# Stanford-ILIAD/PantheonRL

Hardware: AMD Instinct MI355X
Metric: env-steps/sec (all agents) Overcooked-simple PPO self-play (higher is better)
Workload: dtype f32; 1 GPU; OvercookedMultiEnv-v0 layout=simple, PPO self-play (two independent PPO learners per GPU), synthetic (n_envs, n_steps, obs_dim) rollouts; n_envs=1024, n_steps=128, obs_dim=62, features=62, n_logits=6, batch_size=32768, n_epochs=10, agents_per_gpu=2, parallelism=2 agent(s) per gpu x1 gpu(s) = 2 learners (single process), launch_mode=graph, gemm_mode=2, action_masks=none, rollout=scripted, rollout_requested=scripted

## Files before the change

### include/pantheon_hip.h

```cpp
#ifndef PANTHEON_HIP_H
#define PANTHEON_HIP_H

#ifdef __cplusplus
extern "C" {
#endif

#define PH_ABI_VERSION 7
#define PH_HIDDEN 64
#define PH_MAX_COMP 256
#define PH_MAX_LOGITS 64
#define PH_MAX_BOX_ACT 16
#define PH_NSTAT 8
#define PH_MOD_MAX 8
#define PH_MAX_RANKS 16

#define PH_SPACE_BOX 0
#define PH_SPACE_DISCRETE 1

typedef struct ph_ctx ph_ctx;

typedef struct ph_space {
  int kind;
  int n;
  int nvec[PH_MAX_COMP];
// ... 50 lines not shown
int ph_ctx_create(int device, ph_ctx **out );
int ph_ctx_destroy(ph_ctx *ctx);
int ph_ctx_set_stream(ph_ctx *ctx, void *hip_stream );
int ph_ctx_sync(ph_ctx *ctx);
int ph_graph_begin(ph_ctx *ctx);
int ph_graph_end(ph_ctx *ctx, int *graph_id_out );
int ph_graph_launch(ph_ctx *ctx, int graph_id);
int ph_graph_nodes(ph_ctx *ctx, int graph_id, int *nodes_out );
int ph_ctx_set_rng_epoch(ph_ctx *ctx, unsigned long long *epoch_dev );
int ph_rng_epoch_advance(ph_ctx *ctx);
int ph_debug_set_profile_buffer(ph_ctx *ctx, long long *stamps_dev);
int ph_debug_weight_image_mismatches(ph_ctx *ctx, const ph_spec *spec, const float *params, int *mismatches);
int ph_set_exclusive_device(ph_ctx *ctx, int exclusive);
int ph_ctx_step_errors(ph_ctx *ctx, unsigned int *count_out );
int ph_timer_start(ph_ctx *ctx);
int ph_timer_stop(ph_ctx *ctx, float *ms_out );

int ph_layout_of(const ph_spec *spec , ph_layout *out );
int ph_debug_split_tables(const ph_spec *spec, int *slab_map, int *image_map, int *eligible);
int ph_debug_split_oh_tables(const ph_spec *spec, int *slab_map, int *image_map, int *slab_len_out, int *image_elems_out,
                             int *eligible);

int ph_buffer_add(ph_ctx *ctx, const ph_spec *spec, const ph_rollout *rb, int pos, const float *obs ,
                  const float *actions , const float *episode_start ,
                  const float *values , const float *log_probs );
int ph_buffer_add_reward(ph_ctx *ctx, const ph_rollout *rb, int pos, const float *reward ,
                         const unsigned char *env_mask );
int ph_buffer_add_reward_const(ph_ctx *ctx, const ph_rollout *rb, int pos, float reward);
#define PH_JOINT_MATCH_BONUS 0
#define PH_JOINT_RPS 1
int ph_ctx_set_joint_reward_rule(ph_ctx *ctx, int rule);

int ph_buffer_add_reward_joint(ph_ctx *ctx, const ph_rollout *rb, int pos, const float *base_reward ,
                               const int *joint_actions, int n_seats, int seat, const int *partner_seat ,
                               float bonus);
int ph_roundrobin_env_step(ph_ctx *ctx, const int *joint_actions, int *partnerid, const float *base_reward,
                           const float *done, float *reward_out, int *alt_action_out, float *next_block, int block_ld,
                           int n_partners, float bonus, int n);
typedef struct ph_rr_link {
  int n_partners, rank;
  int n, block_ld;
  void *area[PH_MAX_RANKS];
  unsigned long long *error;
  unsigned long long timeout_cycles;
} ph_rr_link;
typedef struct ph_rr_ego {
  const ph_spec *spec;
  const float *params;
  const float *obs_seq;
  const float *base_reward_seq;
  const float *done_seq;
  float *blocks;
  int *partnerid;
  float *rewards;
  int *alt_actions;
  int *partner_trace;
  const float *episode_start0;
  unsigned long long seed, counter0;
  float *values, *log_probs;
  const ph_rollout *rb;
  float bonus;
} ph_rr_ego;
typedef struct ph_rr_partner {
  const ph_spec *spec;
  const float *params;
  float *obs_scratch;
  float *es_scratch;
  unsigned char *can_scratch;
  int *pos;
  unsigned char *boundary, *term, *open, *prev_mask;
  unsigned long long seed, counter0;
  int *actions;
  float *values, *log_probs;
  const ph_rollout *rb;
} ph_rr_partner;
int ph_rr_area_bytes(int n_partners, int n, int block_ld, size_t *bytes_out );
int ph_roundrobin_ego_iteration(ph_ctx *ctx, const ph_rr_link *link, const ph_rr_ego *ego, int T, unsigned long long iteration);
int ph_roundrobin_partner_iteration(ph_ctx *ctx, const ph_rr_link *link, const ph_rr_partner *partner, int T,
                                    unsigned long long iteration);
int ph_buffer_reset(ph_ctx *ctx, const ph_spec *spec, const ph_rollout *rb);

int ph_gae(ph_ctx *ctx, const ph_rollout *rb, const float *last_values , const float *dones ,
           double gamma, double gae_lambda, int mode);

int ph_policy_forward(ph_ctx *ctx, const ph_spec *spec, const float *params, const float *obs, int n,
                      const unsigned char *action_mask, const float *uniforms, const float *given_actions,
                      unsigned long long seed, unsigned long long counter, int deterministic, int *actions_i32,
                      float *actions_f32, float *values, float *log_probs, float *entropy, float *logits,
                      const ph_rollout *rb, int pos, const float *episode_start_in, const float *pending_reward,
                      int gemm_mode);

int ph_policy_act_host(ph_ctx *ctx, const ph_spec *spec, const float *params, const float *obs_host, int n,
                       const float *episode_start_host, unsigned long long seed, unsigned long long counter,
                       int deterministic, int *actions_host, float *values_host, float *log_probs_host,
                       const ph_rollout *rb, int pos, int gemm_mode);

typedef struct ph_step_call {
  const ph_spec *spec;
  const float *params;
  const float *obs;
  int n;
  const unsigned char *action_mask;
  unsigned long long seed, counter;
  int deterministic;
  int *actions_i32;
  float *values;
  float *log_probs;
  const ph_rollout *rb;
  int pos;
  const float *episode_start_in;
  const float *pending_reward;
  const int *joint_actions;
  int n_seats, seat;
  const int *partner_seat;
  float bonus;
} ph_step_call;
#define PH_STEP_FIX_ILLEGAL 2
#define PH_STEP_MASK_ENV_ONLY 4
int ph_policy_step_multi(ph_ctx *ctx, int n_calls, const ph_step_call *calls );

#define PH_COMM_ID_BYTES 128
int ph_comm_unique_id(unsigned char *id_out );
int ph_comm_init(ph_ctx *ctx, const unsigned char *id , int world, int rank);
int ph_comm_destroy(ph_ctx *ctx);
int ph_all_gather_i32(ph_ctx *ctx, const int *local , int *joint , int count);
int ph_selfplay_rollout(ph_ctx *ctx, int n_calls, const ph_step_call *calls , int T,
                        const int *local, int *joint, int count);

#define PH_IPC_HANDLE_BYTES 64
typedef struct ph_p2p {
  int world, rank, count, T;
  int *joint[2][PH_MAX_RANKS];
  unsigned long long *flags[PH_MAX_RANKS];
  unsigned long long *ll[PH_MAX_RANKS];
  int ll_slots;
  const unsigned long long *epoch;
  unsigned long long *error;
  unsigned long long timeout_cycles;
} ph_p2p;
int ph_p2p_alloc(ph_ctx *ctx, size_t bytes, void **ptr_out, unsigned char *handle_out );
int ph_p2p_open(ph_ctx *ctx, const unsigned char *handle , void **ptr_out);
int ph_p2p_close(ph_ctx *ctx, void *ptr);
int ph_p2p_free(ph_ctx *ctx, void *ptr);
int ph_p2p_push(ph_ctx *ctx, const ph_p2p *x, const int *local, int t);
int ph_p2p_wait(ph_ctx *ctx, const ph_p2p *x, int t);
int ph_p2p_ll_push(ph_ctx *ctx, const ph_p2p *x, const int *local, int t);
int ph_p2p_ll_unpack(ph_ctx *ctx, const ph_p2p *x, int t);
int ph_selfplay_rollout_p2p(ph_ctx *ctx, int n_calls, const ph_step_call *calls , int T,
                            const int *local, const ph_p2p *x);

typedef struct ph_rollout_call {
  const ph_spec *spec;
  const float *params;
  const float *obs_seq;
  const float *rew_seq;
  const float *done_seq;
  const unsigned char *mask_seq;
  int n;
  const float *episode_start0;
  unsigned long long seed, counter0;
  int mask_mode;
  int *actions_i32;
  float *values;
  float *log_probs;
  const ph_rollout *rb;
  int n_seats, seat;
// ... 460 lines not shown
```

### pantheonrl_amd/_native.py

```python
from __future__ import annotations

import ctypes as C
import os
from typing import Optional, Sequence

PH_HIDDEN = 64
PH_MAX_COMP = 256
PH_MAX_LOGITS = 64
PH_MAX_BOX_ACT = 16
PH_NSTAT = 8
PH_SPACE_BOX = 0
PH_SPACE_DISCRETE = 1
STAT_NAMES = ("policy_loss", "value_loss", "entropy_loss", "clip_fraction", "approx_kl", "loss", "grad_norm", "applied")

_HERE = os.path.dirname(os.path.abspath(__file__))
LIB_PATH = os.environ.get("PANTHEON_HIP_LIB") or os.path.join(_HERE, "csrc", "libpantheon_hip.so")


class NativeError(RuntimeError):
    """Raised for any non-zero status from the C ABI (message from ph_last_error)."""


class PhSpace(C.Structure):
    _fields_ = [("kind", C.c_int), ("n", C.c_int), ("nvec", C.c_int * PH_MAX_COMP)]
# ... 191 lines not shown
                ("log_probs", C.c_void_p), ("seed", C.c_ulonglong)]


class PhLiarPool(C.Structure):
    _fields_ = [("n", C.c_int), ("spec", C.POINTER(PhSpec)),
                ("hands", C.c_void_p), ("history", C.c_void_p), ("nmoves", C.c_void_p), ("ego_first", C.c_void_p),
                ("dice_seed", C.c_ulonglong), ("probegostart", C.c_float),
                ("ego_params", C.c_void_p), ("ego_rb", C.POINTER(PhRollout)), ("ego_actions", C.c_void_p),
                ("ego_values", C.c_void_p), ("ego_log_probs", C.c_void_p), ("ego_episode_start", C.c_void_p),
                ("ego_seed", C.c_ulonglong),
                ("members", C.POINTER(PhPoolMember)), ("n_members", C.c_int), ("partnerid", C.c_void_p),
                ("resample", C.c_int), ("pool_seed", C.c_ulonglong),
                ("alt_actions", C.c_void_p), ("alt_acted", C.c_void_p),
                ("obs_ego", C.c_void_p), ("obs_alt", C.c_void_p), ("episodes", C.c_void_p),
                ("obs_next", C.c_void_p), ("rew1", C.c_void_p), ("rew2", C.c_void_p), ("es_alt", C.c_void_p),
                ("done1", C.c_void_p), ("done2", C.c_void_p), ("running", C.c_void_p), ("can", C.c_void_p),
                ("alt_opens", C.c_void_p), ("ego_opens", C.c_void_p), ("done", C.c_void_p)]


XPLAY_NSTAT = 4


class PhLiarXplay(C.Structure):
    _fields_ = [("n", C.c_int), ("spec", C.POINTER(PhSpec)),
                ("hands", C.c_void_p), ("history", C.c_void_p), ("nmoves", C.c_void_p), ("ego_first", C.c_void_p),
                ("dice_seed", C.c_ulonglong), ("probegostart", C.c_float),
                ("members", C.POINTER(PhPoolMember)), ("n_members", C.c_int),
                ("pairs", C.POINTER(C.c_int)), ("n_pairs", C.c_int), ("episodes_per_table", C.c_int),
                ("ego_id", C.c_void_p), ("alt_id", C.c_void_p),
                ("ego_actions", C.c_void_p), ("alt_actions", C.c_void_p),
                ("obs_ego", C.c_void_p), ("obs_alt", C.c_void_p),
                ("games", C.c_void_p), ("playing", C.c_void_p), ("tables_left", C.c_void_p),
                ("ep_return", C.c_void_p), ("ep_length", C.c_void_p), ("returns", C.c_void_p), ("lengths", C.c_void_p),
                ("obs_next", C.c_void_p), ("rew1", C.c_void_p), ("rew2", C.c_void_p),
                ("done1", C.c_void_p), ("done2", C.c_void_p), ("running", C.c_void_p),
                ("alt_opens", C.c_void_p), ("ego_opens", C.c_void_p), ("done", C.c_void_p)]


class PhLiarRecord(C.Structure):
    _fields_ = [("n", C.c_int), ("cap", C.c_int), ("rows", C.c_void_p), ("member", C.c_void_p),
                ("count", C.c_void_p), ("count_alt", C.c_void_p), ("dropped", C.c_void_p), ("pending", C.c_void_p)]


RECORD_ROW = 33

EPISODE_NSTAT = 4


class PhEpisodeScan(C.Structure):
    _fields_ = [("rb", C.POINTER(PhRollout)), ("T", C.c_int), ("last_dones", C.c_void_p), ("carry_return", C.c_void_p),
                ("carry_length", C.c_void_p), ("carry_valid", C.c_void_p), ("n_members", C.c_int), ("member", C.c_void_p),
                ("resample", C.c_int), ("pool_seed", C.c_ulonglong), ("counter0", C.c_ulonglong), ("stats", C.c_void_p)]


SIGNATURES = {
    "ph_abi_version": [],
    "ph_roundrobin_env_step": [_vp, _vp, _vp, _vp, _vp, _vp, _vp, _vp, _i, _i, C.c_float, _i],
    "ph_last_error": [],
    "ph_device_count": [C.POINTER(_i)],
    "ph_ctx_create": [_i, C.POINTER(_vp)],
    "ph_ctx_destroy": [_vp],
    "ph_ctx_set_stream": [_vp, _vp],
    "ph_ctx_sync": [_vp],
    "ph_graph_begin": [_vp],
    "ph_graph_end": [_vp, C.POINTER(_i)],
    "ph_graph_launch": [_vp, _i],
    "ph_graph_nodes": [_vp, _i, C.POINTER(C.c_int)],
    "ph_ctx_set_rng_epoch": [_vp, _vp],
    "ph_rng_epoch_advance": [_vp],
    "ph_debug_set_profile_buffer": [_vp, _vp],
    "ph_set_exclusive_device": [_vp, _i],
    "ph_ctx_step_errors": [_vp, C.POINTER(C.c_uint)],
    "ph_debug_weight_image_mismatches": [_vp, C.POINTER(PhSpec), _vp, C.POINTER(C.c_int)],
    "ph_timer_start": [_vp],
    "ph_timer_stop": [_vp, C.POINTER(C.c_float)],
    "ph_layout_of": [C.POINTER(PhSpec), C.POINTER(PhLayout)],
    "ph_debug_split_tables": [C.POINTER(PhSpec), C.POINTER(C.c_int), C.POINTER(C.c_int), C.POINTER(C.c_int)],
    "ph_debug_split_oh_tables": [C.POINTER(PhSpec), _vp, _vp, C.POINTER(_i), C.POINTER(_i), C.POINTER(_i)],
    "ph_buffer_add": [_vp, C.POINTER(PhSpec), C.POINTER(PhRollout), _i, _vp, _vp, _vp, _vp, _vp],
    "ph_buffer_add_reward": [_vp, C.POINTER(PhRollout), _i, _vp, _vp],
    "ph_buffer_add_reward_joint": [_vp, C.POINTER(PhRollout), _i, _vp, _vp, _i, _i, _vp, C.c_float],
    "ph_buffer_reset": [_vp, C.POINTER(PhSpec), C.POINTER(PhRollout)],
    "ph_gae": [_vp, C.POINTER(PhRollout), _vp, _vp, _d, _d, _i],
    "ph_policy_forward": [_vp, C.POINTER(PhSpec), _vp, _vp, _i, _vp, _vp, _vp, _ull, _ull, _i, _vp, _vp, _vp, _vp, _vp,
                          _vp, C.POINTER(PhRollout), _i, _vp, _vp, _i],
    "ph_ctx_set_joint_reward_rule": [_vp, _i],
    "ph_adapmult_layout_of": [C.POINTER(PhSpec), _i, _vp],
    "ph_adapmult_forward": [_vp, C.POINTER(PhSpec), _i, _vp, _vp, _i, _vp, _vp, _vp, _ull, _ull, _i, _vp, _vp, _vp, _vp, _vp,
                            _vp, C.POINTER(PhRollout), _i, _vp],
    "ph_adapmult_minibatch_grad": [_vp, C.POINTER(PhSpec), _i, _vp, C.POINTER(PhRollout), C.POINTER(PhPpoHyper), _vp, _i, _vp, _vp,
                                   _vp],
    "ph_adapmult_train": [_vp, C.POINTER(PhSpec), _i, C.POINTER(PhOptState), C.POINTER(PhRollout), C.POINTER(PhPpoHyper), _i, _i,
                          _vp, _ull, _vp, _vp],
    "ph_policy_act_host": [_vp, C.POINTER(PhSpec), _vp, _vp, _i, _vp, _ull, _ull, _i, _vp, _vp, _vp, C.POINTER(PhRollout), _i, _i],
    "ph_buffer_add_reward_const": [_vp, C.POINTER(PhRollout), _i, C.c_float],
    "ph_policy_step_multi": [_vp, _i, C.POINTER(PhStepCall)],
    "ph_policy_forward_ragged": [_vp, C.POINTER(PhSpec), _vp, _vp, _vp, _ull, _ull, _i, _vp, _vp, _vp, C.POINTER(PhRollout),
                                 _vp, _vp, _vp],
    "ph_buffer_add_reward_ragged": [_vp, C.POINTER(PhRollout), _vp, _vp, _vp],
    "ph_ragged_advance": [_vp, C.POINTER(PhRollout), _vp, _vp],
    "ph_buffer_compact_columns": [_vp, C.POINTER(PhSpec), C.POINTER(PhRollout), C.POINTER(PhRollout), _vp, _i],
    "ph_fix_illegal_actions": [_vp, _vp, _vp, _i, _i],
    "ph_rps_step": [_vp, _vp, _vp, _vp, _vp, _i],
    "ph_liar_step": [_vp, _vp, _vp, _vp, _vp, _vp, _vp, _vp, _vp, _vp, _i],
    "ph_liar_reset": [_vp, _vp, _vp, _vp, _vp, _vp, _ull, _ull, C.c_float, _i],
    "ph_liar_obs": [_vp, _vp, _vp, _vp, _vp, _vp, _vp, _i],
    "ph_liar_selfplay_step": [_vp, C.POINTER(PhLiarSelfPlay), _i, _ull, _i],
    "ph_liar_selfplay_rollout": [_vp, C.POINTER(PhLiarSelfPlay), _i, _i, _ull],
    "ph_pool_forward": [_vp, C.POINTER(PhSpec), C.POINTER(PhPoolMember), _i, _vp, _vp, _vp, _ull, _vp, _vp, _i],
    "ph_liar_default_actions": [_vp, _vp, _vp, _vp, _i],
    "ph_liar_pool_step": [_vp, C.POINTER(PhLiarPool), _i, _ull, _i],
    "ph_liar_xplay_step": [_vp, C.POINTER(PhLiarXplay), _ull, _i],
    "ph_xplay_stats": [_vp, _vp, _vp, _vp, _i, _i, _i, _vp],
    "ph_episode_stats": [_vp, C.POINTER(PhEpisodeScan)],
    "ph_liar_record_attach": [_vp, C.POINTER(PhLiarRecord)],
    "ph_liar_record_export": [_vp, C.POINTER(PhLiarRecord), _i, _vp, _vp, _vp, C.c_longlong],
    "ph_block_reset": [_vp, _i, _vp, _vp, _ull, _ull, _i],
    "ph_block_step": [_vp, _i, _vp, _vp, _i, _vp, _vp, _vp, _vp, _i],
    "ph_block_obs": [_vp, _i, _vp, _i, _vp, _vp, _i],
    "ph_block_selfplay_step": [_vp, C.POINTER(PhBlockSelfPlay), _i, _ull],
    "ph_block_replay_host": [_i, _i, _i, _vp, _vp, _vp, _vp, _vp, _vp, _vp, _i, _ull, _ull, _i],
    "ph_framestack_push": [_vp, _vp, _vp, _vp, _vp, _i, _i, _i],
    "ph_scripted_rollout": [_vp, C.POINTER(PhSpec), _vp, _vp, _vp, _vp, _i, _i, _vp, _ull, _ull, _vp, _vp, _vp,
                            C.POINTER(PhRollout), _i, _i],
    "ph_ppo_train": [_vp, C.POINTER(PhSpec), C.POINTER(PhOptState), C.POINTER(PhRollout), C.POINTER(PhPpoHyper), _i, _i,
                     _vp, _ull, _vp, _i],
    "ph_ppo_train_multi": [C.POINTER(PhTrainCall), _i],
    "ph_comm_unique_id": [_vp],
    "ph_comm_init": [_vp, _vp, _i, _i],
    "ph_comm_destroy": [_vp],
    "ph_all_gather_i32": [_vp, _vp, _vp, _i],
    "ph_selfplay_rollout": [_vp, _i, C.POINTER(PhStepCall), _i, _vp, _vp, _i],
    "ph_p2p_alloc": [_vp, C.c_size_t, C.POINTER(C.c_void_p), _vp],
    "ph_p2p_open": [_vp, _vp, C.POINTER(C.c_void_p)],
    "ph_p2p_close": [_vp, _vp],
    "ph_p2p_free": [_vp, _vp],
    "ph_p2p_push": [_vp, C.POINTER(PhP2P), _vp, _i],
    "ph_p2p_wait": [_vp, C.POINTER(PhP2P), _i],
    "ph_p2p_ll_push": [_vp, C.POINTER(PhP2P), _vp, _i],
    "ph_p2p_ll_unpack": [_vp, C.POINTER(PhP2P), _i],
    "ph_selfplay_rollout_p2p": [_vp, _i, C.POINTER(PhStepCall), _i, _vp, C.POINTER(PhP2P)],
    "ph_selfplay_rollout_persistent": [_vp, _i, C.POINTER(PhRolloutCall), _i, C.POINTER(PhP2P), _i],
    "ph_selfplay_rollout_persistent_capacity": [_vp, C.POINTER(_i)],
    "ph_rr_area_bytes": [_i, _i, _i, C.POINTER(C.c_size_t)],
    "ph_roundrobin_ego_iteration": [_vp, C.POINTER(PhRRLink), C.POINTER(PhRREgo), _i, _ull],
    "ph_roundrobin_partner_iteration": [_vp, C.POINTER(PhRRLink), C.POINTER(PhRRPartner), _i, _ull],
    "ph_modular_layout": [C.POINTER(PhSpec), C.POINTER(PhModular), C.POINTER(PhLayout), C.POINTER(PhLayout), C.POINTER(_i)],
    "ph_modular_forward": [_vp, C.POINTER(PhSpec), C.POINTER(PhModular), _vp, _i, _vp, _i, _vp, _vp, _vp, _ull, _ull, _i, _vp,
                           _vp, _vp, _vp, _vp, _vp, _vp, C.POINTER(PhRollout), _i, _vp, _vp, _i],
    "ph_modular_train": [_vp, C.POINTER(PhSpec), C.POINTER(PhModular), C.POINTER(PhOptState), _vp, C.POINTER(PhRollout),
                         C.POINTER(PhPpoHyper), _i, _i, _vp, _ull, _vp, C.c_float, _i],
    "ph_modular_minibatch_grad": [_vp, C.POINTER(PhSpec), C.POINTER(PhModular), _vp, _i, C.POINTER(PhRollout),
                                  C.POINTER(PhPpoHyper), _vp, _i, C.c_float, _vp, _vp, _i],
    "ph_ppo_minibatch_grad": [_vp, C.POINTER(PhSpec), _vp, C.POINTER(PhRollout), C.POINTER(PhPpoHyper), _vp, _i, _vp,
                              _vp, _i],
    "ph_adap_train": [_vp, C.POINTER(PhSpec), C.POINTER(PhOptState), C.POINTER(PhRollout), C.POINTER(PhPpoHyper), _i, _i,
                      _vp, _ull, _vp, _i, C.POINTER(PhAdapLoss)],
    "ph_adap_minibatch_grad": [_vp, C.POINTER(PhSpec), _vp, C.POINTER(PhRollout), C.POINTER(PhPpoHyper), _vp, _i, _vp,
                               _vp, _i, C.POINTER(PhAdapLoss)],
    "ph_bench_ppo_grad": [_vp, C.POINTER(PhSpec), _vp, C.POINTER(PhRollout), C.POINTER(PhPpoHyper), _i, _i, _i,
                          C.POINTER(C.c_float)],
    "ph_bench_gae": [_vp, C.POINTER(PhRollout), _vp, _vp, _d, _d, _i, _i, C.POINTER(C.c_float)],
    "ph_bench_train_kernels": [_vp, C.POINTER(PhSpec), C.POINTER(PhOptState), C.POINTER(PhRollout), C.POINTER(PhPpoHyper),
                               _i, _i, _i, _i, C.POINTER(C.c_float)],
    "ph_feistel_indices": [_i, _ull, _i, _i, _i, C.POINTER(_i)],
    "ph_arch_layout_of": [C.POINTER(PhSpec), C.POINTER(PhArch), C.POINTER(PhArchLayout)],
# ... 247 lines not shown
```

### pantheonrl_amd/csrc/ph_abi.hip

```cpp
#include <dlfcn.h>
#include <hip/hip_runtime.h>
#include <rccl/rccl.h>

#include <atomic>
#include <chrono>
#include <cmath>
#include <cstdio>
#include <cstdint>
#include <cstring>
#include <mutex>
#include <string>
#include <vector>

#include "ph_launch.h"
#include "ph_block.h"
#include "ph_arch.h"
#include "ph_pool.h"
#include "ph_xplay.h"
#include "ph_record.h"
#include "ph_episode.h"
#include "ph_adap_vec.h"

namespace ph {

// ... 38 lines not shown
  const bool slot = dev >= 0 && dev < 64;
  int cu = slot ? cached[dev].load(std::memory_order_relaxed) : 0;
  if (cu > 0) return cu;
  if (hipDeviceGetAttribute(&cu, hipDeviceAttributeMultiprocessorCount, dev) != hipSuccess || cu <= 0) return 0;
  if (slot) cached[dev].store(cu, std::memory_order_relaxed);
  return cu;
}

}

namespace {

thread_local std::string g_err;

int fail(const std::string& m) {
  g_err = m;
  return 1;
}
int fail_hip(const char* what, hipError_t e) {
  g_err = std::string(what) + ": " + hipGetErrorString(e);
  return 2;
}
#define PH_HIP(call)                                   \
  do {                                                 \
    hipError_t _e = (call);                            \
    if (_e != hipSuccess) return fail_hip(#call, _e);  \
  } while (0)

struct SpecCache {
  ph_spec spec;
  int* obs_off = nullptr;
  int* act_off = nullptr;
  int* slab_map = nullptr;
  int* slab_map_split = nullptr;
  int* wimage_map = nullptr;
  int split_kind = 0;
  int slab_len_split = 0;
  int wimage_elems = 0;
  int id = 0;
};

}

struct ph_ctx {
  int device = 0;
  hipStream_t stream = nullptr;
  float* slabs = nullptr;
  size_t slabs_cap = 0;
  float* statpart = nullptr;
  size_t statpart_cap = 0;
  float* grad = nullptr;
  size_t grad_cap = 0;
  float* blocksq = nullptr;
  size_t blocksq_cap = 0;
  float* advstats = nullptr;
  size_t advstats_cap = 0;
  ph::AdamBias* adam_bias = nullptr;
  size_t adam_bias_cap = 0;
  float* act_stage_host = nullptr;
  float* act_stage_dev = nullptr;
  size_t act_stage_cap = 0;
  unsigned int* act_done_host = nullptr;
  unsigned int* act_done_dev = nullptr;
  unsigned int act_seq = 0;
  unsigned int* fwd_host_done = nullptr;
  int joint_reward_rule = 0;
  int wimage_zeroed_for = 0;
  size_t wimage_cap = 0;
  bool exclusive = false;
  unsigned short* wimage = nullptr;
  double* advpart = nullptr;
  size_t advpart_cap = 0;
  int* perm_idx = nullptr;
  size_t perm_idx_cap = 0;
  int* perm_phys = nullptr;
  size_t perm_phys_cap = 0;
  uint4* ximg = nullptr;
  size_t ximg_cap = 0;
  uint4* rec_pi = nullptr;
  uint4* rec_vf = nullptr;
  size_t rec_cap = 0;
  uint4* rowrec = nullptr;
  size_t rowrec_cap = 0;
  unsigned long long* step_words = nullptr;
  size_t step_words_cap = 0;
  unsigned int* step_gen = nullptr;
  float* am_buf = nullptr;
  size_t am_buf_cap = 0;
  float* adap_extra = nullptr;
  size_t adap_extra_cap = 0;
  float* adap_loss = nullptr;
  size_t adap_loss_cap = 0;
  float* scalars = nullptr;
  int* stop_flag = nullptr;
  std::vector<SpecCache> specs;
  std::vector<hipGraphExec_t> graphs;
  std::vector<int> graph_nodes;
  bool capturing = false;
  hipEvent_t ev0 = nullptr, ev1 = nullptr;
  ph_p2p* p2p_dev = nullptr;
  ph_p2p p2p_host;
  bool p2p_valid = false;
  void* comm = nullptr;
  int comm_world = 1, comm_rank = 0;
  hipEvent_t ev_grad = nullptr;
  int num_cu = 256;
  int exchange_blocks_per_cu = 0;
  unsigned long long* rng_epoch = nullptr;
  ph::RecordLog rec{};
  bool recording = false;
  ph::PoolMemberDev* pool_dev = nullptr;
  ph::PoolMemberDev pool_host[PH_MAX_POOL];
  int pool_count = 0;
  bool pool_wide = false;
  size_t pool_tower_lds = 0;
  bool pool_adap = false;
  int* pool_order = nullptr;
  size_t pool_order_cap = 0;
  int* pool_tiles = nullptr;
  size_t pool_tiles_cap = 0;
  long long* prof = nullptr;
  double* ep_partial = nullptr;
  size_t ep_partial_cap = 0;
  unsigned int* ep_ticket = nullptr;
  struct ModWs {
    float* act = nullptr;
    size_t act_cap = 0;
    int* maps = nullptr;
    ph_spec spec;
    ph_modular mod;
    bool maps_valid = false;
    float* kl_sum = nullptr;
    int* scratch = nullptr;
  } mw;
};

namespace {

struct DevGuard {
  int prev = -1;
  bool switched = false;
  explicit DevGuard(const ph_ctx* ctx) {
    if (!ctx) return;
    if (hipGetDevice(&prev) == hipSuccess && prev != ctx->device) switched = hipSetDevice(ctx->device) == hipSuccess;
  }
  ~DevGuard() {
    if (switched) (void)hipSetDevice(prev);
  }
  DevGuard(const DevGuard&) = delete;
  DevGuard& operator=(const DevGuard&) = delete;
};

template <typename T>
int ensure(const ph_ctx* ctx, T*& p, size_t& cap, size_t n) {
  if (n <= cap) return 0;
  if (ctx->capturing) return fail("workspace would grow inside graph capture: run the same call once outside capture first");
  if (p) (void)hipFree(p);
  p = nullptr;
  cap = 0;
  hipError_t e = hipMalloc((void**)&p, n * sizeof(T));
  if (e != hipSuccess) return fail_hip("hipMalloc(workspace)", e);
  cap = n;
  return 0;
}

int check_space(const ph_space& s, const char* name) {
// ... 153 lines not shown
int arch_host_dims(const ph_spec* spec, const ph_arch* arch, ph::NetDims* nd, ph::ArchDims* ad);
int arch_lds_refusal(const ph::NetDims& nd, const ph::ArchDims& ad);

int fwd_args(ph::FwdArgs& a, ph_ctx* ctx, const ph_spec* spec, bool box_act_ok, const float* params, const float* obs, int n,
             unsigned long long seed, unsigned long long counter, int* act_i32, float* values, float* logp,
             const ph_arch* arch = nullptr, ph::ArchDims* ad = nullptr) {
  std::memset(&a, 0, sizeof(a));
  if (arch ? arch_resolve(ctx, spec, arch, &a.nd, ad) : resolve(ctx, spec, &a.nd, box_act_ok)) return 1;
  a.params = params;
  a.obs = obs;
  a.n = n;
  a.seed = seed;
  a.counter = counter;
  a.epoch = ctx->rng_epoch;
  a.act_i32 = act_i32;
  a.values = values;
  a.logp = logp;
  return 0;
}

int fwd_bind_row(const char* who, ph::FwdArgs& a, const ph_rollout* rb, int pos, const float* episode_start_in,
                 const float* pending_reward) {
  if (!rb) return pending_reward ? fail_who(who, ": pending_reward needs the fused rollout-buffer write") : 0;
  if (check_rb(rb)) return 1;
  if (a.n != rb->E) return fail_who(who, ": fused add needs n == rollout E");
  if (pos < 0 || pos >= rb->T) return fail_who(who, ": pos out of range (buffer full?)");
  if (!episode_start_in) return fail_who(who, ": fused add needs episode_start_in");
  const size_t row = (size_t)pos * rb->E;
  a.rb_obs = rb->observations + row * a.nd.D;
  a.rb_act = rb->actions + row * a.nd.A;
  a.rb_rew = rb->rewards + row;
  a.rb_es = rb->episode_starts + row;
  a.rb_val = rb->values + row;
  a.rb_logp = rb->log_probs + row;
  a.es_in = episode_start_in;
  if (pending_reward) {
    if (pos < 1) return fail_who(who, ": pending_reward needs pos >= 1");
    a.prev_rew = rb->rewards + (row - rb->E);
    a.pending_reward = pending_reward;
  }
  return 0;
}
void fwd_bind_bases(ph::FwdArgs& a, const ph_rollout* rb, const float* es_in, const int* pos_env, const unsigned char* rec_mask) {
  a.rb_obs = rb->observations;
  a.rb_act = rb->actions;
  a.rb_rew = rb->rewards;
  a.rb_es = rb->episode_starts;
  a.rb_val = rb->values;
  a.rb_logp = rb->log_probs;
  a.es_in = es_in;
  if (!pos_env) return;
  a.pos_env = pos_env;
  a.rec_mask = rec_mask;
  a.rb_T = rb->T;
}

void fwd_eval_fields(ph::FwdArgs& a, const unsigned char* mask, const float* uniforms, const float* given_actions, int deterministic,
                     float* act_f32, float* entropy, float* logits) {
  a.mask = mask;
  a.uniforms = uniforms;
  a.given_actions = given_actions;
  a.deterministic = deterministic;
  a.act_f32 = act_f32;
  a.entropy = entropy;
  a.logits = logits;
}

int forward_run(const char* who, ph_ctx* ctx, const ph_spec* spec, const ph_arch* arch, const float* params, const float* obs, int n,
                const unsigned char* action_mask, const float* uniforms, const float* given_actions, unsigned long long seed,
                unsigned long long counter, int deterministic, int* actions_i32, float* actions_f32, float* values, float* log_probs,
                float* entropy, float* logits, const ph_rollout* rb, int pos, const float* episode_start_in,
                const float* pending_reward, int gemm_mode) {
  if (!ctx) return fail("null ctx");
  if (!params || !obs) return fail_who(who, ": null params/obs");
  if ((uintptr_t)params % 16 != 0) return fail_who(who, ": params must be 16-byte aligned");
  if (n <= 0) return fail_who(who, ": n must be positive");
  ph::FwdArgs a;
  ph::ArchDims ad;
  if (fwd_args(a, ctx, spec, true, params, obs, n, seed, counter, actions_i32, values, log_probs, arch, &ad)) return 1;
  if (a.nd.gauss && action_mask) return fail_who(who, ": action masks belong to the categorical heads");
  fwd_eval_fields(a, action_mask, uniforms, given_actions, deterministic, actions_f32, entropy, logits);
  a.prof = ctx->prof;
  if (fwd_bind_row(who, a, rb, pos, episode_start_in, pending_reward)) return 1;
  if (arch) {
    PH_HIP(ph::launch_arch_fwd(a, ad, gemm_mode, ctx->stream));
    return 0;
  }
  a.host_done = ctx->fwd_host_done;
  a.host_seq = ctx->act_seq;
  PH_HIP(ph::launch_policy_fwd(a, gemm_mode, ctx->stream));
  return 0;
}

int forward_ragged_run(const char* who, ph_ctx* ctx, const ph_spec* spec, const ph_arch* arch, const float* params, const float* obs,
                       const unsigned char* action_mask, unsigned long long seed, unsigned long long counter, int deterministic,
                       int* actions_i32, float* values, float* log_probs, const ph_rollout* rb, const int* pos_env,
                       const unsigned char* record_mask, const float* episode_start_in, int gemm_mode) {
  if (!ctx) return fail("null ctx");
  if (!params || !obs || !pos_env || !record_mask || !episode_start_in) return fail_who(who, ": null argument");
  if ((uintptr_t)params % 16 != 0) return fail_who(who, ": params must be 16-byte aligned");
  if (check_rb(rb)) return 1;
  ph::FwdArgs a;
  ph::ArchDims ad;
  if (fwd_args(a, ctx, spec, false, params, obs, rb->E, seed, counter, actions_i32, values, log_probs, arch, &ad)) return 1;
  a.mask = action_mask;
  a.prof = ctx->prof;
  a.deterministic = deterministic;
  fwd_bind_bases(a, rb, episode_start_in, pos_env, record_mask);
  PH_HIP(arch ? ph::launch_arch_fwd(a, ad, gemm_mode, ctx->stream) : ph::launch_policy_fwd(a, gemm_mode, ctx->stream));
  return 0;
}

int scripted_rollout_run(const char* who, ph_ctx* ctx, const ph_spec* spec, const ph_arch* arch, const float* params,
                         const float* obs_seq, const float* rew_seq, const float* done_seq, int n, int n_steps,
                         const float* episode_start0, unsigned long long seed, unsigned long long counter0, int* actions_i32,
                         float* values, float* log_probs, const ph_rollout* rb, int pos0, int gemm_mode) {
  if (!ctx) return fail("null ctx");
  if (!params || !obs_seq || !rew_seq || !done_seq || !episode_start0) return fail_who(who, ": null argument");
  if ((uintptr_t)params % 16 != 0) return fail_who(who, ": params must be 16-byte aligned");
  if (n <= 0 || n_steps <= 0) return fail_who(who, ": n and n_steps must be positive");
  if (check_rb(rb)) return 1;
  if (n != rb->E) return fail_who(who, ": n must equal the rollout buffer's E");
  if (pos0 < 0 || pos0 > rb->T - n_steps) return fail_who(who, ": rows pos0 .. pos0 + n_steps - 1 must lie in the buffer");
  ph::FwdArgs a;
  ph::ArchDims ad;
  if (fwd_args(a, ctx, spec, false, params, obs_seq, n, seed, counter0, actions_i32, values, log_probs, arch, &ad)) return 1;
  if (!arch && !ph::fwd16_eligible(a.nd, n))
    return fail_who(who, ": needs the 16-row forward's shape class (one feature chunk, one Discrete head of <= 8 logits, "
                         "n < 16384); use ph_policy_forward per step");
  a.prof = ctx->prof;
  if (fwd_bind_row(who, a, rb, pos0, episode_start0, nullptr)) return 1;
  ph::ScriptedSteps sc;
  std::memset(&sc, 0, sizeof(sc));
  sc.n_steps = n_steps;
  sc.obs_seq = obs_seq;
  sc.rew_seq = rew_seq;
  sc.done_seq = done_seq;
  PH_HIP(arch ? ph::launch_arch_rollout(a, ad, sc, gemm_mode, ctx->stream)
              : ph::launch_policy_fwd16_rollout(a, sc, gemm_mode, ctx->stream));
  return 0;
}

ph::AdvStatArgs adv_args_epochs(const ph_ctx* ctx, const ph_rollout* rb, const int* perms, unsigned long long perm_seed, int batch,
                                int n_mb) {
  const int N = rb->T * rb->E;
  ph::AdvStatArgs aa{};
  aa.rb_adv = rb->advantages;
  aa.T = rb->T;
  aa.E = rb->E;
  aa.perms = perms;
  aa.perm_n = (uint32_t)N;
  aa.perm_hb = ph::feistel_half_bits((uint32_t)N);
  aa.perm_seed = perm_seed;
  aa.epoch = ctx->rng_epoch;
  aa.N = N;
  aa.batch = batch;
  aa.n_mb = n_mb;
  aa.out = ctx->advstats;
  aa.partial = ctx->advpart;
  aa.idx_out = perms ? nullptr : ctx->perm_idx;
  aa.phys_out = ctx->perm_phys;
  return aa;
}
ph::AdvStatArgs adv_args_minibatch(const ph_ctx* ctx, const ph_rollout* rb, const int* indices, int nb) {
  ph::AdvStatArgs aa{};
  aa.rb_adv = rb->advantages;
  aa.T = rb->T;
  aa.E = rb->E;
  aa.perms = indices;
  aa.perm_hb = 1;
  aa.N = nb;
  aa.batch = nb;
  aa.n_mb = 1;
  aa.out = ctx->advstats;
  aa.partial = ctx->advpart;
  aa.phys_out = ctx->perm_phys;
  return aa;
}

struct MbWalk {
  int ep, start, nb;
  const int* idx;
};
MbWalk minibatch_walk(const ph_ctx* ctx, const int* perms, int N, int n_mb, int batch_size, int mbi) {
  MbWalk w;
  w.ep = mbi / n_mb;
  w.start = (mbi - w.ep * n_mb) * batch_size;
  w.nb = N - w.start < batch_size ? N - w.start : batch_size;
  w.idx = (perms ? perms : ctx->perm_idx) + (size_t)w.ep * N + w.start;
  return w;
}

ph::ReduceArgs reduce_args(const ph_ctx* ctx, const ph_ppo_hyper* hp, const ph_opt_state* opt, int P, int slab_len, const int* map,
                           int nslab, int nb, float* grad, float* stats_out) {
  ph::ReduceArgs r;
  r.slabs = ctx->slabs;
  r.nslab = nslab;
  r.nstatpart = 2 * nslab;
  r.P = P;
  r.slab_len = slab_len;
  r.map = map;
  r.grad = grad;
  r.blocksq = ctx->blocksq;
  r.statpart = ctx->statpart;
  r.stats_out = stats_out;
  r.nb = nb;
  r.ent_coef = hp->ent_coef;
  r.vf_coef = hp->vf_coef;
  r.target_kl = opt ? hp->target_kl : -1.f;
  r.stop_flag = ctx->stop_flag;
  r.step = opt ? opt->step : nullptr;
  r.scalars = ctx->scalars;
  return r;
}
ph::AdamArgs adam_args(const ph_ctx* ctx, const ph_ppo_hyper* hp, const ph_opt_state* opt, int P, int slab_len, float* stats_out,
                       unsigned short* wimage, const int* wimage_map) {
  ph::AdamArgs ad;
  ad.params = opt->params;
  ad.m = opt->adam_m;
  ad.v = opt->adam_v;
// ... 450 lines not shown
    es.joint = slot;
    es.partnerid = ego->partnerid;
    es.partner_trace = ego->partner_trace ? ego->partner_trace + (size_t)t * n : nullptr;
    es.base = ego->base_reward_seq + (size_t)t * n;
    es.done = ego->done_seq + (size_t)t * n;
    es.reward_out = ego->rewards + (size_t)t * n;
    es.alt_action_out = ego->alt_actions ? ego->alt_actions + (size_t)t * n : nullptr;
    es.next_block = ego->blocks + (size_t)((t + 1) % T) * n * ld;
    es.block_ld = ld;
    es.n_partners = K;
    es.n = n;
    es.bonus = ego->bonus;
    PH_HIP(ph::launch_rr_env_step(es, ctx->stream));
  }
  return 0;
}

int ph_roundrobin_partner_iteration(ph_ctx* ctx, const ph_rr_link* link, const ph_rr_partner* pa, int T,
                                    unsigned long long iteration) {
  DevGuard dev_guard(ctx);
  if (!ctx || !pa || T <= 0) return fail("ph_roundrobin_partner_iteration: bad argument");
  if (check_rr_link(link)) return 1;
  if (link->rank < 1) return fail("ph_roundrobin_partner_iteration: partners live on ranks 1 .. n_partners");
  if (!pa->params || !pa->es_scratch || !pa->can_scratch || !pa->pos || !pa->boundary || !pa->term ||
      !pa->open || !pa->prev_mask || !pa->actions || !pa->values || !pa->log_probs || !pa->rb)
    return fail("ph_roundrobin_partner_iteration: null argument");
  if (check_rb(pa->rb)) return 1;
  if (pa->rb->E != link->n) return fail("ph_roundrobin_partner_iteration: the rollout buffer must have one column per environment");
  const int n = link->n, k = link->rank - 1;
  for (int t = 0; t < T; ++t) {
    const unsigned long long want = iteration * (unsigned long long)T + (unsigned long long)t + 1ull;
    ph::RRPartnerStep st;
    std::memset(&st, 0, sizeof(st));
    st.block_stamp = rr_stamps(link, link->rank);
    st.act_stamp = rr_stamps(link, 0) + 1 + k;
    st.want = want;
    st.timeout = link->timeout_cycles;
    st.error = link->error;
    st.block = (const float*)rr_slot(link, link->rank, t & 1);
    st.block_ld = link->block_ld;
    st.n = n;
    st.T = pa->rb->T;
    st.k = k;
    st.rewards = pa->rb->rewards;
    st.pos = pa->pos;
    st.boundary = pa->boundary;
    st.term = pa->term;
    st.open = pa->open;
    st.prev_mask = pa->prev_mask;
    st.can = pa->can_scratch;
    st.es = pa->es_scratch;
    st.actions = pa->actions;
    st.act_dst = (int*)rr_slot(link, 0, t & 1) + (size_t)(1 + k) * n;
    PH_HIP(ph::launch_rr_partner_pre(st, ctx->stream));
    const float* obs_t = st.block + (size_t)n * 4;
    if (ph_policy_forward_ragged(ctx, pa->spec, pa->params, obs_t, nullptr, pa->seed, pa->counter0 + (unsigned long long)t,
                                 0, pa->actions, pa->values, pa->log_probs, pa->rb, pa->pos, pa->can_scratch, pa->es_scratch))
      return 1;
    PH_HIP(ph::launch_rr_partner_post(st, ctx->stream));
  }
  return 0;
}

int ph_buffer_reset(ph_ctx* ctx, const ph_spec* spec, const ph_rollout* rb) {
  DevGuard dev_guard(ctx);
  if (!ctx) return fail("null ctx");
  ph_layout lay;
  if (layout_of(spec, &lay) || check_rb(rb)) return 1;
  const size_t n = (size_t)rb->T * rb->E;
  PH_HIP(hipMemsetAsync(rb->observations, 0, n * lay.D * sizeof(float), ctx->stream));
  PH_HIP(hipMemsetAsync(rb->actions, 0, n * lay.A * sizeof(float), ctx->stream));
  float* arrs[] = {rb->rewards, rb->episode_starts, rb->values, rb->log_probs, rb->advantages, rb->returns};
  for (float* a : arrs) PH_HIP(hipMemsetAsync(a, 0, n * sizeof(float), ctx->stream));
  return 0;
}

int ph_gae(ph_ctx* ctx, const ph_rollout* rb, const float* last_values, const float* dones, double gamma,
           double gae_lambda, int mode) {
  DevGuard dev_guard(ctx);
  if (!ctx) return fail("null ctx");
  if (check_rb(rb)) return 1;
  if (!last_values || !dones) return fail("ph_gae: null last_values/dones");
  if (mode < 0 || mode > 2) return fail("ph_gae: mode must be 0, 1 or 2");
  PH_HIP(ph::launch_gae(rb->rewards, rb->values, rb->episode_starts, last_values, dones, rb->advantages, rb->returns,
                        rb->T, rb->E, gamma, gae_lambda, mode, ctx->stream));
  return 0;
}

int ph_policy_forward(ph_ctx* ctx, const ph_spec* spec, const float* params, const float* obs, int n,
                      const unsigned char* action_mask, const float* uniforms, const float* given_actions,
                      unsigned long long seed, unsigned long long counter, int deterministic, int* actions_i32,
                      float* actions_f32, float* values, float* log_probs, float* entropy, float* logits,
                      const ph_rollout* rb, int pos, const float* episode_start_in, const float* pending_reward,
                      int gemm_mode) {
  DevGuard dev_guard(ctx);
  return forward_run("ph_policy_forward", ctx, spec, nullptr, params, obs, n, action_mask, uniforms, given_actions, seed, counter,
                     deterministic, actions_i32, actions_f32, values, log_probs, entropy, logits, rb, pos, episode_start_in,
                     pending_reward, gemm_mode);
}

int ph_policy_act_host(ph_ctx* ctx, const ph_spec* spec, const float* params, const float* obs_host, int n,
                       const float* episode_start_host, unsigned long long seed, unsigned long long counter, int deterministic,
                       int* actions_host, float* values_host, float* log_probs_host, const ph_rollout* rb, int pos, int gemm_mode) {
  DevGuard dev_guard(ctx);
  if (!ctx) return fail("null ctx");
  if (!params || !obs_host) return fail("ph_policy_act_host: null params/obs");
  if (n <= 0) return fail("ph_policy_act_host: n must be positive");
  if (rb && !episode_start_host) return fail("ph_policy_act_host: the fused rollout-buffer write needs episode_start_host");
  if (ctx->capturing) return fail("ph_policy_act_host synchronises: not inside graph capture");
  ph::NetDims nd;
  if (resolve(ctx, spec, &nd)) return 1;
  const size_t n_in = (size_t)n * nd.D + (size_t)n, n_out = (size_t)n * nd.A + 2 * (size_t)n, need = n_in + n_out;
  if (need > ctx->act_stage_cap) {
    if (ctx->act_stage_host) (void)hipHostFree(ctx->act_stage_host);
    ctx->act_stage_host = nullptr;
    ctx->act_stage_dev = nullptr;
    ctx->act_stage_cap = 0;
    const size_t cap = need < 4096 ? 4096 : need;
    PH_HIP(hipHostMalloc((void**)&ctx->act_stage_host, cap * sizeof(float), hipHostMallocMapped | hipHostMallocCoherent));
    PH_HIP(hipHostGetDevicePointer((void**)&ctx->act_stage_dev, ctx->act_stage_host, 0));
    ctx->act_stage_cap = cap;
  }
  float *h = ctx->act_stage_host, *d = ctx->act_stage_dev;
  std::memcpy(h, obs_host, (size_t)n * nd.D * sizeof(float));
  if (episode_start_host) std::memcpy(h + (size_t)n * nd.D, episode_start_host, (size_t)n * sizeof(float));
  else std::memset(h + (size_t)n * nd.D, 0, (size_t)n * sizeof(float));
  float* d_out = d + n_in;
  int* d_act = reinterpret_cast<int*>(d_out);
  float *d_val = d_out + (size_t)n * nd.A, *d_lp = d_val + n;
  const bool words = n <= 16 && ph::fwd16_eligible(nd, n);
  if (words && !ctx->act_done_host) {
    PH_HIP(hipHostMalloc((void**)&ctx->act_done_host, 64, hipHostMallocMapped | hipHostMallocCoherent));
    PH_HIP(hipHostGetDevicePointer((void**)&ctx->act_done_dev, ctx->act_done_host, 0));
    ctx->act_done_host[0] = ctx->act_done_host[1] = 0;
  }
  if (words) {
    if (++ctx->act_seq == 0) ctx->act_seq = 1;
    ctx->fwd_host_done = ctx->act_done_dev;
  }
  const int frc = ph_policy_forward(ctx, spec, params, d, n, nullptr, nullptr, nullptr, seed, counter, deterministic, d_act,
                                    nullptr, d_val, d_lp, nullptr, nullptr, rb, pos, rb ? d + (size_t)n * nd.D : nullptr, nullptr,
                                    gemm_mode);
  ctx->fwd_host_done = nullptr;
  if (frc) return 1;
  bool arrived = false;
  if (words) {
    const unsigned int seq = ctx->act_seq;
    const auto t0 = std::chrono::steady_clock::now();
    for (unsigned spins = 0;; ++spins) {
      if (__atomic_load_n(ctx->act_done_host, __ATOMIC_ACQUIRE) == seq &&
          __atomic_load_n(ctx->act_done_host + 1, __ATOMIC_ACQUIRE) == seq) {
        arrived = true;
        break;
      }
      if ((spins & 1023) == 1023 && std::chrono::steady_clock::now() - t0 > std::chrono::milliseconds(50)) break;
      __builtin_ia32_pause();
    }
  }
  if (!arrived) PH_HIP(hipStreamSynchronize(ctx->stream));
  const float* h_out = h + n_in;
  if (actions_host) std::memcpy(actions_host, h_out, (size_t)n * nd.A * sizeof(int));
  if (values_host) std::memcpy(values_host, h_out + (size_t)n * nd.A, (size_t)n * sizeof(float));
  if (log_probs_host) std::memcpy(log_probs_host, h_out + (size_t)n * nd.A + n, (size_t)n * sizeof(float));
  return 0;
}

int ph_scripted_rollout(ph_ctx* ctx, const ph_spec* spec, const float* params, const float* obs_seq, const float* rew_seq,
                        const float* done_seq, int n, int n_steps, const float* episode_start0, unsigned long long seed,
// ... 1278 lines not shown
                  " is not a multiple of 32 in [32, PH_ARCH_MAX_WIDTH (256)]");
  std::memset(o, 0, sizeof(*o));
  o->D = base.D; o->F = base.F; o->A = base.A; o->L = base.L;
  long long off = 0;
  for (int net = 0; net < 2; ++net) {
    int in = base.F;
    for (int l = 0; l < arch->n_layers; ++l) {
      const int w = arch->width[l];
      (net == 0 ? o->pi_W : o->vf_W)[l] = (int)off; off += (long long)in * w;
      (net == 0 ? o->pi_b : o->vf_b)[l] = (int)off; off += w;
      in = w;
    }
  }
  const int wn = arch->width[arch->n_layers - 1];
  o->act_W = (int)off; off += (long long)wn * base.L;
  o->act_b = (int)off; off += base.L;
  o->val_W = (int)off; off += wn;
  o->val_b = (int)off; off += 1;
  if (off >= (1ll << 31)) return fail("ph_arch: parameter count must fit in int32");
  o->P = (int)off;
  return 0;
}

int arch_lds_refusal(const ph::NetDims& nd, const ph::ArchDims& ad) {
  const size_t need = std::max(ph::arch_grad_lds_bytes(nd, ad, ph::ARCH_FWD_ROWS), ph::arch_fwd_lds_bytes(nd, ad));
  if (need > ph::ARCH_LDS_MAX)
    return fail("ph_arch: observation space too large for the tower kernels' LDS tile (" + std::to_string(need) +
                " bytes at 32 rows, " + std::to_string(ph::ARCH_LDS_MAX) + " available)");
  return 0;
}

int arch_host_dims(const ph_spec* spec, const ph_arch* arch, ph::NetDims* nd, ph::ArchDims* ad) {
  std::memset(ad, 0, sizeof(*ad));
  if (arch_layout(spec, arch, &ad->lay)) return 1;
  ad->nl = arch->n_layers;
  for (int l = 0; l < arch->n_layers; ++l) ad->w[l] = arch->width[l];
  std::memset(nd, 0, sizeof(*nd));
  nd->obs_kind = spec->obs.kind;
  nd->D = ad->lay.D;
  nd->nchunk = (ad->lay.F + PH_HIDDEN - 1) / PH_HIDDEN;
  return 0;
}

int arch_resolve(ph_ctx* ctx, const ph_spec* spec, const ph_arch* arch, ph::NetDims* nd, ph::ArchDims* ad) {
  std::memset(ad, 0, sizeof(*ad));
  if (arch_layout(spec, arch, &ad->lay)) return 1;
  if (resolve(ctx, spec, nd, false)) return 1;
  ad->nl = arch->n_layers;
  for (int l = 0; l < arch->n_layers; ++l) ad->w[l] = arch->width[l];
  nd->slab_map = nd->slab_map_split = nd->wimage_map = nullptr;
  nd->split = nd->split_kind = 0;
  nd->lay.P = ad->lay.P;
  return arch_lds_refusal(*nd, *ad);
}

void fill_grad_args(ph::GradArgs& g, const ph::NetDims& nd, const float* params, const ph_rollout* rb,
                    const ph_ppo_hyper* hp, ph_ctx* ctx) {
  g.nd = nd;
  g.params = params;
  g.rb_obs = rb->observations;
  g.rb_act = rb->actions;
  g.rb_val = rb->values;
  g.rb_logp = rb->log_probs;
  g.rb_adv = rb->advantages;
  g.rb_ret = rb->returns;
  g.T = rb->T;
  g.E = rb->E;
  g.clip = hp->clip_range;
  g.clip_vf = hp->clip_range_vf;
  g.ent_coef = hp->ent_coef;
  g.vf_coef = hp->vf_coef;
  g.norm_adv = hp->normalize_advantage;
  g.slabs = ctx->slabs;
  g.statpart = ctx->statpart;
  g.stop_flag = ctx->stop_flag;
  g.prof = ctx->prof;
  g.wimage = ctx->wimage;
  g.ximg = ctx->ximg;
  g.ximg_zero_row = rb->T * rb->E;
  g.rec_pi = ctx->rec_pi;
  g.rec_vf = ctx->rec_vf;
}

int rebuild_weight_image(ph_ctx* ctx, const ph::NetDims& nd, const float* params) {
  if (!nd.split) return 0;
  if ((size_t)nd.wimage_elems > ctx->wimage_cap) {
    if (ctx->capturing) return fail("first split-kernel use inside graph capture: call it once outside capture first");
    if (ensure(ctx, ctx->wimage, ctx->wimage_cap, (size_t)nd.wimage_elems)) return 1;
    ctx->wimage_zeroed_for = 0;
  }
  if (ctx->wimage_zeroed_for != nd.spec_id) {
    if (ctx->capturing) return fail("the weight image changes its spec inside graph capture: run the same call once outside capture first");
    PH_HIP(hipMemsetAsync(ctx->wimage, 0, (size_t)nd.wimage_elems * sizeof(unsigned short), ctx->stream));
    ctx->wimage_zeroed_for = nd.spec_id;
  }
  PH_HIP(ph::launch_weight_image(params, ctx->wimage, nd.wimage_map, nd.lay.P, ctx->stream));
  return 0;
}

int build_grad_pack(ph_ctx* ctx, const ph::NetDims& nd, const ph_rollout* rb, size_t n_rec) {
  if (nd.split != 1) return 0;
  const size_t rows = (size_t)rb->T * rb->E;
  const size_t need_img = (rows + 1) * ph::XIMG_ROW_U4;
  if (ensure(ctx, ctx->ximg, ctx->ximg_cap, need_img)) return 1;
  if (ensure(ctx, ctx->rowrec, ctx->rowrec_cap, 2 * rows)) return 1;
  if (n_rec > ctx->rec_cap) {
    size_t c1 = ctx->rec_cap, c2 = ctx->rec_cap;
    if (ensure(ctx, ctx->rec_pi, c1, n_rec)) return 1;
    if (ensure(ctx, ctx->rec_vf, c2, n_rec)) return 1;
    ctx->rec_cap = n_rec;
  }
  PH_HIP(ph::launch_obs_planes(rb->observations, (int)rows, nd.D, nd.F, ph::grad_fast_fold(nd) ? 1 : 0, ctx->ximg, rb->advantages,
                               rb->log_probs, rb->actions, rb->returns, rb->values, ctx->rowrec, ctx->stream));
  return 0;
}
void fill_adv_records(ph::AdvStatArgs& aa, const ph_ctx* ctx, const ph::NetDims& nd, const ph_rollout* rb) {
  aa.rec_pi_out = nd.split == 1 ? ctx->rec_pi : nullptr;
  aa.rec_vf_out = nd.split == 1 ? ctx->rec_vf : nullptr;
  aa.rowrec = (nd.split == 1 && rb->advantages && rb->log_probs && rb->actions && rb->returns && rb->values) ? ctx->rowrec : nullptr;
  aa.rb_logp = rb->log_probs;
  aa.rb_act = rb->actions;
  aa.rb_ret = rb->returns;
  aa.rb_val = rb->values;
}


void select_gemm(ph::NetDims& nd, int gemm_mode) {
  nd.split = (gemm_mode == 2 && nd.slab_map_split != nullptr) ? nd.split_kind : 0;
  if (nd.split) nd.slab_map = nd.slab_map_split;
}

int slab_len_of(const ph::NetDims& nd) { return nd.split ? nd.slab_len_split : (nd.slab_map ? 2 * ph::RS_NET : nd.lay.P); }

int ensure_train_ws(ph_ctx* ctx, int P, int slab_len, int nwg_max, int n_mb_total, size_t n_idx = 0, size_t n_phys = 0) {
  if (n_phys && ensure(ctx, ctx->perm_phys, ctx->perm_phys_cap, n_phys)) return 1;
  if (ensure(ctx, ctx->slabs, ctx->slabs_cap, (size_t)nwg_max * slab_len)) return 1;
  if (ensure(ctx, ctx->statpart, ctx->statpart_cap, (size_t)2 * nwg_max * ph::NSTATP)) return 1;
  if (ensure(ctx, ctx->grad, ctx->grad_cap, (size_t)P)) return 1;
  if (ensure(ctx, ctx->blocksq, ctx->blocksq_cap, (size_t)ph::reduce_blocks(slab_len))) return 1;
  if (ensure(ctx, ctx->advstats, ctx->advstats_cap, (size_t)n_mb_total * 2)) return 1;
  if (ensure(ctx, ctx->adam_bias, ctx->adam_bias_cap, (size_t)n_mb_total)) return 1;
  if (ensure(ctx, ctx->advpart, ctx->advpart_cap, (size_t)n_mb_total * 2 * ph::ADV_SPLIT)) return 1;
  if (n_idx && ensure(ctx, ctx->perm_idx, ctx->perm_idx_cap, n_idx)) return 1;
  const size_t n_words = (size_t)ph::reduce_blocks(slab_len) + 1;
  if (n_words > ctx->step_words_cap) {
    if (ensure(ctx, ctx->step_words, ctx->step_words_cap, n_words)) return 1;
    PH_HIP(hipMemsetAsync(ctx->step_words, 0, n_words * sizeof(unsigned long long), ctx->stream));
  }
  if (!ctx->step_gen) {
    if (ctx->capturing) return fail("workspace would grow inside graph capture: run the same call once outside capture first");
    PH_HIP(hipMalloc((void**)&ctx->step_gen, 4 * sizeof(unsigned int)));
    PH_HIP(hipMemsetAsync(ctx->step_gen, 0, 4 * sizeof(unsigned int), ctx->stream));
  }
  return 0;
}

bool step_fused_wanted(const ph_ctx* ctx, int slab_len, bool alone) {
  return alone && ctx->exclusive && ctx->step_words && ctx->step_gen &&
         ph::step_fused_fits(ph::reduce_blocks(slab_len), slab_len, ctx->num_cu);
}

}

namespace {

struct TrainPlan {
  int alone = 1;
  ph_ctx* ctx;
  ph::NetDims nd;
  const ph_opt_state* opt;
  const ph_rollout* rb;
  const ph_ppo_hyper* hp;
  const int* perms;
  unsigned long long perm_seed;
  float* stats;
  int n_epochs, batch_size, gemm_mode, N, n_mb, P;
  uint32_t hb;
  const ph_adap_loss* adap = nullptr;
  bool arch = false;
  ph::ArchDims arch_dims;
};

int adap_check(ph_ctx* ctx, const ph::NetDims& nd, const ph_adap_loss* ad, const char* who) {
  const std::string w(who);
  if (nd.obs_kind != PH_SPACE_BOX) return fail(w + ": the context term needs Box observations (observation ++ context)");
  if (ad->context_size <= 0 || ad->context_size >= nd.F) return fail(w + ": context_size must be in (0, observation length)");
  if (ad->num_context_samples < 2 || ad->num_context_samples > ph::ADAP_ROWS)
    return fail(w + ": num_context_samples must be in [2, 16]");
  if (ad->num_state_samples <= 0) return fail(w + ": num_state_samples must be positive");
  if (ad->sampler < PH_CTX_L2 || ad->sampler > PH_CTX_NATURAL_NUMBERS) return fail(w + ": unknown context sampler");
  if (ad->sampler == PH_CTX_NATURAL_NUMBERS && ad->context_size != 1)
    return fail(w + ": the natural_numbers sampler draws (num, 1) contexts: context_size must be 1");
  if (ph::adap_lds_bytes(nd, ad->num_context_samples, ad->context_size) > 160 * 1024)
    return fail(w + ": observation / action space too large for the context kernel's LDS tile");
  const size_t nwg = (size_t)ph::adap_workgroups(ad->num_context_samples, ad->num_state_samples);
  if (ensure(ctx, ctx->adap_extra, ctx->adap_extra_cap, nwg * ph::adap_slab_floats(nd.lay))) return 1;
  if (ensure(ctx, ctx->adap_loss, ctx->adap_loss_cap, nwg)) return 1;
  return 0;
}

int adap_launch(ph_ctx* ctx, const ph::NetDims& nd, const float* params, const ph_rollout* rb, const ph_adap_loss* ad,
                const int* idx, int nb, int mbi, ph::ReduceArgs* r) {
  const int C = ad->num_context_samples, S = ad->num_state_samples, cs = ad->context_size;
  const int n_states = S < nb ? S : nb;
  const int nwg = ph::adap_workgroups(C, n_states);
  ph::AdapArgs a;
  std::memset(&a, 0, sizeof(a));
  a.nd = nd;
  a.params = params;
  a.rb_obs = rb->observations;
  a.T = rb->T;
  a.E = rb->E;
  a.idx = idx;
  a.nb = nb;
  a.ctx_size = cs;
  a.n_ctx = C;
  a.n_states = n_states;
  a.sampler = ad->sampler;
  a.coef = ad->context_loss_coeff;
  a.state_idx = ad->state_idx ? ad->state_idx + (size_t)mbi * S : nullptr;
  a.contexts = ad->contexts ? ad->contexts + (size_t)mbi * C * cs : nullptr;
  a.seed = ad->seed;
  a.epoch = ctx->rng_epoch;
  a.mbi = (uint32_t)mbi;
  a.nb_hb = ph::feistel_half_bits((uint32_t)nb);
  a.extra = ctx->adap_extra;
  a.loss_part = ctx->adap_loss;
  a.used_state_idx = ad->used_state_idx ? ad->used_state_idx + (size_t)mbi * S : nullptr;
  a.used_contexts = ad->used_contexts ? ad->used_contexts + (size_t)mbi * C * cs : nullptr;
  a.stop_flag = ctx->stop_flag;
  a.prof = ctx->prof;
  PH_HIP(ph::launch_adap_context(a, nwg, ctx->stream));
  r->extra = ctx->adap_extra;
  r->n_extra = nwg;
  r->extra_len = ph::adap_slab_floats(nd.lay);
  r->extra_cut = nd.lay.vf_W1;
  r->extra_lo = nd.lay.act_W;
  r->extra_hi = nd.lay.val_W;
  r->extra_loss = ctx->adap_loss;
  r->extra_norm = 1.0f / (float)((C * (C - 1) / 2) * n_states);
  r->extra_coef = ad->context_loss_coeff;
  r->extra_loss_out = ad->context_loss ? ad->context_loss + mbi : nullptr;
  return 0;
}

void train_adv_args(const TrainPlan& t, bool need_idx, ph::AdvStatArgs& aa) {
  aa = adv_args_epochs(t.ctx, t.rb, t.perms, t.perm_seed, t.batch_size, t.n_mb);
  aa.clear_flag = t.ctx->stop_flag;
  if (t.nd.split == 1 && !need_idx) aa.idx_out = aa.phys_out = nullptr;
  fill_adv_records(aa, t.ctx, t.nd, t.rb);
  aa.adam_bias = t.ctx->adam_bias;
  aa.opt_step = t.opt->step;
  aa.lr = t.hp->learning_rate;
  aa.beta1 = t.hp->adam_beta1;
  aa.beta2 = t.hp->adam_beta2;
}

int train_prepare(const char* who, TrainPlan& t, ph_ctx* ctx, const ph_spec* spec, const ph_opt_state* opt, const ph_rollout* rb,
                  const ph_ppo_hyper* hp, int n_epochs, int batch_size, const int* perms, unsigned long long perm_seed,
                  float* stats, int gemm_mode, bool need_idx = false, const ph_arch* arch = nullptr) {
  if (check_train_call(who, ctx, opt, hp, n_epochs, batch_size) || check_rb(rb)) return 1;
  t.arch = arch != nullptr;
  if (arch) {
    if (arch_resolve(ctx, spec, arch, &t.nd, &t.arch_dims)) return 1;
  } else {
    if (resolve(ctx, spec, &t.nd, true)) return 1;
    select_gemm(t.nd, gemm_mode);
  }
  t.ctx = ctx;
  t.opt = opt;
  t.rb = rb;
  t.hp = hp;
  t.perms = perms;
  t.perm_seed = perm_seed;
  t.stats = stats;
  t.n_epochs = n_epochs;
  t.batch_size = batch_size;
  t.gemm_mode = gemm_mode;
  t.N = rb->T * rb->E;
  t.n_mb = (t.N + batch_size - 1) / batch_size;
  t.P = t.nd.lay.P;
  const MbPlan big = plan_minibatch(ctx, t.nd, batch_size < t.N ? batch_size : t.N, t.arch ? &t.arch_dims : nullptr);
  if (ensure_train_ws(ctx, t.P, slab_len_of(t.nd), big.nwg, n_epochs * t.n_mb, perms ? 0 : (size_t)n_epochs * t.N,
                      (size_t)n_epochs * t.N))
    return 1;
  hipStream_t s = ctx->stream;
  if (rebuild_weight_image(ctx, t.nd, opt->params)) return 1;
  if (build_grad_pack(ctx, t.nd, rb, (size_t)n_epochs * t.N)) return 1;
  t.hb = ph::feistel_half_bits((uint32_t)t.N);
  ph::AdvStatArgs aa;
  train_adv_args(t, need_idx, aa);
  PH_HIP(ph::launch_adv_stats(aa, n_epochs * t.n_mb, s));
  return 0;
}

void fill_step_args(const TrainPlan& t, int mbi, const MbPlan& pl, ph::ReduceArgs& r, ph::AdamArgs& ad);
constexpr unsigned long long STEP_WAIT_TICKS = 200000000ull;

int train_launch_grad(const TrainPlan& t, int mbi, MbPlan* pl_out) {
  ph_ctx* ctx = t.ctx;
  const MbWalk w = minibatch_walk(ctx, t.perms, t.N, t.n_mb, t.batch_size, mbi);
  const size_t pos = (size_t)w.ep * t.N + w.start;
  const MbPlan pl = plan_minibatch(ctx, t.nd, w.nb, t.arch ? &t.arch_dims : nullptr);
  ph::GradArgs g;
  std::memset(&g, 0, sizeof(g));
  fill_grad_args(g, t.nd, t.opt->params, t.rb, t.hp, ctx);
  g.idx = w.idx;
  g.idx_phys = ctx->perm_phys + pos;
  if (t.nd.split == 1) {
    g.rec_pi = ctx->rec_pi + pos;
    g.rec_vf = ctx->rec_vf + pos;
  }
  g.perm_n = (uint32_t)t.N;
  g.perm_hb = t.hb;
  g.perm_seed = t.perm_seed;
  g.perm_epoch = w.ep;
  g.epoch = ctx->rng_epoch;
  g.mb_start = w.start;
  g.nb = w.nb;
  g.advstats = ctx->advstats + 2 * (size_t)mbi;
  g.ntiles = pl.ntiles;
  *pl_out = pl;
  if (t.arch) PH_HIP(ph::launch_arch_grad(g, t.arch_dims, pl.nwg, t.gemm_mode, ctx->stream));
  else PH_HIP(ph::launch_ppo_grad(g, pl.nwg, t.gemm_mode, ctx->stream));
  return 0;
}

void fill_step_args(const TrainPlan& t, int mbi, const MbPlan& pl, ph::ReduceArgs& r, ph::AdamArgs& ad) {
  ph_ctx* ctx = t.ctx;
  float* stats_out = t.stats ? t.stats + (size_t)mbi * PH_NSTAT : nullptr;
  r = reduce_args(ctx, t.hp, t.opt, t.P, slab_len_of(t.nd), t.nd.slab_map, pl.nwg, pl.nb, ctx->grad, stats_out);
  r.wide = t.alone && ctx->exclusive;
  ad = adam_args(ctx, t.hp, t.opt, t.P, slab_len_of(t.nd), stats_out, t.nd.split ? ctx->wimage : nullptr, t.nd.wimage_map);
  ad.bias = ctx->adam_bias + mbi;
}

int train_launch_step(const TrainPlan& t, int mbi, const MbPlan& pl) {
  ph_ctx* ctx = t.ctx;
  hipStream_t s = ctx->stream;
  ph::ReduceArgs r;
  ph::AdamArgs ad;
  fill_step_args(t, mbi, pl, r, ad);
  if (t.adap) {
    const MbWalk w = minibatch_walk(ctx, t.perms, t.N, t.n_mb, t.batch_size, mbi);
    if (adap_launch(ctx, t.nd, t.opt->params, t.rb, t.adap, w.idx, w.nb, mbi, &r)) return 1;
  }
  if (step_fused_wanted(ctx, slab_len_of(t.nd), t.alone != 0)) {
    PH_HIP(ph::launch_ppo_step(r, ad, ctx->step_words, ctx->step_gen, ctx->step_gen + 1, STEP_WAIT_TICKS, s));
  } else {
    PH_HIP(ph::launch_ppo_reduce(r, s));
    PH_HIP(ph::launch_ppo_adam(ad, s));
  }
  return 0;
}

}

namespace {
int train_run(const char* who, ph_ctx* ctx, const ph_spec* spec, const ph_opt_state* opt, const ph_rollout* rb,
              const ph_ppo_hyper* hp, int n_epochs, int batch_size, const int* perms, unsigned long long perm_seed, float* stats,
              int gemm_mode, const ph_adap_loss* adap, const ph_arch* arch = nullptr) {
  TrainPlan t;
  if (train_prepare(who, t, ctx, spec, opt, rb, hp, n_epochs, batch_size, perms, perm_seed, stats, gemm_mode, adap != nullptr, arch))
    return 1;
  if (adap && t.nd.gauss) return fail("ph_adap_train: the context term is written for the categorical heads");
  if (adap && adap_check(ctx, t.nd, adap, "ph_adap_train")) return 1;
  t.adap = adap;
  for (int mbi = 0; mbi < n_epochs * t.n_mb; ++mbi) {
    MbPlan pl;
    if (train_launch_grad(t, mbi, &pl)) return 1;
    if (train_launch_step(t, mbi, pl)) return 1;
  }
  return 0;
}
}

int ph_ppo_train(ph_ctx* ctx, const ph_spec* spec, const ph_opt_state* opt, const ph_rollout* rb,
                 const ph_ppo_hyper* hp, int n_epochs, int batch_size, const int* perms,
                 unsigned long long perm_seed, float* stats, int gemm_mode) {
  DevGuard dev_guard(ctx);
  return train_run("ph_ppo_train", ctx, spec, opt, rb, hp, n_epochs, batch_size, perms, perm_seed, stats, gemm_mode, nullptr);
}

int ph_adap_train(ph_ctx* ctx, const ph_spec* spec, const ph_opt_state* opt, const ph_rollout* rb,
                  const ph_ppo_hyper* hp, int n_epochs, int batch_size, const int* perms,
                  unsigned long long perm_seed, float* stats, int gemm_mode, const ph_adap_loss* adap) {
  DevGuard dev_guard(ctx);
  if (!adap) return fail("ph_adap_train: null context-term description");
  return train_run("ph_adap_train", ctx, spec, opt, rb, hp, n_epochs, batch_size, perms, perm_seed, stats, gemm_mode, adap);
}

int ph_ppo_train_multi(const ph_train_call* calls, int n_calls) {
  if (!calls || n_calls <= 0) return fail("ph_ppo_train_multi: no calls");
  if (n_calls > PH_MAX_TRAIN_CALLS) return fail("ph_ppo_train_multi: too many calls");
  TrainPlan t[PH_MAX_TRAIN_CALLS];
  int total[PH_MAX_TRAIN_CALLS], longest = 0;
  for (int k = 0; k < n_calls; ++k) {
    const ph_train_call& c = calls[k];
    if (train_prepare("ph_ppo_train_multi", t[k], c.ctx, c.spec, c.opt, c.rb, c.hyper, c.n_epochs, c.batch_size, c.perms,
                      c.perm_seed, c.stats, c.gemm_mode))
      return 1;
    t[k].alone = n_calls == 1;
    if (!t[k].ctx->ev_grad) PH_HIP(hipEventCreateWithFlags(&t[k].ctx->ev_grad, hipEventDisableTiming));
    total[k] = c.n_epochs * t[k].n_mb;
    longest = total[k] > longest ? total[k] : longest;
  }
  hipEvent_t prev = nullptr;
  hipStream_t prev_stream = nullptr;
  for (int mbi = 0; mbi < longest; ++mbi) {
    for (int k = 0; k < n_calls; ++k) {
      if (mbi >= total[k]) continue;
      hipStream_t s = t[k].ctx->stream;
      if (prev && prev_stream != s) PH_HIP(hipStreamWaitEvent(s, prev, 0));
      MbPlan pl;
      if (train_launch_grad(t[k], mbi, &pl)) return 1;
      PH_HIP(hipEventRecord(t[k].ctx->ev_grad, s));
      prev = t[k].ctx->ev_grad;
      prev_stream = s;
      if (train_launch_step(t[k], mbi, pl)) return 1;
    }
  }
  return 0;
}

namespace {
int minibatch_grad_run(const char* who, ph_ctx* ctx, const ph_spec* spec, const float* params, const ph_rollout* rb,
                       const ph_ppo_hyper* hp, const int* indices, int nb, float* grad_out, float* stats_out, int gemm_mode,
                       const ph_adap_loss* adap, const ph_arch* arch = nullptr);
}

int ph_ppo_minibatch_grad(ph_ctx* ctx, const ph_spec* spec, const float* params, const ph_rollout* rb,
                          const ph_ppo_hyper* hp, const int* indices, int nb, float* grad_out, float* stats_out,
                          int gemm_mode) {
  DevGuard dev_guard(ctx);
  return minibatch_grad_run("ph_ppo_minibatch_grad", ctx, spec, params, rb, hp, indices, nb, grad_out, stats_out, gemm_mode, nullptr);
}

int ph_adap_minibatch_grad(ph_ctx* ctx, const ph_spec* spec, const float* params, const ph_rollout* rb,
                           const ph_ppo_hyper* hp, const int* indices, int nb, float* grad_out, float* stats_out,
                           int gemm_mode, const ph_adap_loss* adap) {
  DevGuard dev_guard(ctx);
  if (!adap) return fail("ph_adap_minibatch_grad: null context-term description");
  return minibatch_grad_run("ph_adap_minibatch_grad", ctx, spec, params, rb, hp, indices, nb, grad_out, stats_out, gemm_mode, adap);
}

namespace {
int minibatch_grad_run(const char* who, ph_ctx* ctx, const ph_spec* spec, const float* params, const ph_rollout* rb,
                       const ph_ppo_hyper* hp, const int* indices, int nb, float* grad_out, float* stats_out, int gemm_mode,
                       const ph_adap_loss* adap, const ph_arch* arch) {
  if (check_minibatch_call(who, ctx, params, rb, hp, indices, nb, grad_out)) return 1;
  ph::NetDims nd;
  ph::ArchDims ad;
  if (arch) {
    if (arch_resolve(ctx, spec, arch, &nd, &ad)) return 1;
  } else {
    if (resolve(ctx, spec, &nd, adap == nullptr)) return 1;
    select_gemm(nd, gemm_mode);
  }
  const int P = nd.lay.P;
  const MbPlan pl = plan_minibatch(ctx, nd, nb, arch ? &ad : nullptr);
  if (ensure_train_ws(ctx, P, slab_len_of(nd), pl.nwg, 1, 0, (size_t)nb)) return 1;
  hipStream_t s = ctx->stream;
  PH_HIP(ph::launch_set_int(ctx->stop_flag, 0, s));
  if (rebuild_weight_image(ctx, nd, params)) return 1;
// ... 954 lines not shown
```

### pantheonrl_amd/csrc/ph_gae.hip

```cpp
#include "ph_launch.h"

namespace ph {

__global__ __launch_bounds__(64) void gae_serial_kernel(const float* __restrict__ rew, const float* __restrict__ val,
                                                        const float* __restrict__ es, const float* __restrict__ last_values,
                                                        const float* __restrict__ dones, float* __restrict__ adv,
                                                        float* __restrict__ ret, int T, int E, float g, float gl) {
#pragma clang fp contract(off)
  const int e = blockIdx.x * blockDim.x + threadIdx.x;
  if (e >= E) return;
  float nv = last_values[e];
  float nnt = 1.0f - dones[e];
  float last = 0.f;
  int t = T - 1;
  for (; t >= 7; t -= 8) {
    float r[8], v[8], s[8];
#pragma unroll
    for (int u = 0; u < 8; ++u) {
      const size_t o = (size_t)(t - u) * E + e;
      r[u] = rew[o];
      v[u] = val[o];
      s[u] = es[o];
    }
#pragma unroll
    for (int u = 0; u < 8; ++u) {
      const size_t o = (size_t)(t - u) * E + e;
      const float delta = (r[u] + (g * nv) * nnt) - v[u];
      last = delta + ((gl * nnt) * last);
      adv[o] = last;
      ret[o] = last + v[u];
      nv = v[u];
      nnt = 1.0f - s[u];
    }
  }
  for (; t >= 0; --t) {
    const size_t o = (size_t)t * E + e;
    const float r = rew[o], v = val[o], s = es[o];
    const float delta = (r + (g * nv) * nnt) - v;
    last = delta + ((gl * nnt) * last);
    adv[o] = last;
    ret[o] = last + v;
    nv = v;
    nnt = 1.0f - s;
  }
}

__device__ __forceinline__ float gae_ld(const float* p) { return __builtin_nontemporal_load(p); }
__device__ __forceinline__ void gae_st(float* p, float v) { __builtin_nontemporal_store(v, p); }

template <int LC, int EB>
__global__ __launch_bounds__(1024) void gae_scan_kernel(const float* __restrict__ rew, const float* __restrict__ val,
                                                        const float* __restrict__ es,
                                                        const float* __restrict__ last_values,
                                                        const float* __restrict__ dones, float* __restrict__ adv,
                                                        float* __restrict__ ret, int T, int E, int NCH, float g,
                                                        float gl) {
  extern __shared__ __attribute__((aligned(16))) float sm[];
  float* sS = sm;
  float* sP = sm + NCH * EB;
  float* carry = sP + NCH * EB;
  const int el = threadIdx.x % EB, ch = threadIdx.x / EB;
  const int e = blockIdx.x * EB + el;
  const bool env_ok = e < E;
  const int span = NCH * LC;
  if (ch == 0) carry[el] = 0.f;
  for (int top = T; top > 0; top -= span) {
    const int base = top - span;
    const int t0 = base + ch * LC;
    const int tend = t0 + LC;
    const bool live = env_ok && tend > 0;
    float a[LC], cp[LC], vv[LC];
    float S = 0.f, P = 1.f;
    if (live) {
      float nv, nnt;
      if (tend == T) {
        nv = last_values[e];
        nnt = 1.0f - dones[e];
      } else {
        nv = val[(size_t)tend * E + e];
        nnt = 1.0f - es[(size_t)tend * E + e];
      }
      float r[LC], s[LC];
#pragma unroll
      for (int k = 0; k < LC; ++k) {
        const int t = t0 + k;
        const size_t o = (size_t)(t >= 0 ? t : 0) * E + e;
        r[k] = gae_ld(rew + o);
        vv[k] = gae_ld(val + o);
        s[k] = gae_ld(es + o);
      }
      float A = 0.f, Pacc = 1.f;
#pragma unroll
      for (int k = LC - 1; k >= 0; --k) {
        if (t0 + k >= 0) {
          const float delta = r[k] + g * nv * nnt - vv[k];
          const float c = gl * nnt;
          A = delta + c * A;
          Pacc = c * Pacc;
          nv = vv[k];
          nnt = 1.0f - s[k];
        }
        a[k] = A;
        cp[k] = Pacc;
      }
      S = A;
      P = Pacc;
    }
    __syncthreads();
    sS[ch * EB + el] = S;
    sP[ch * EB + el] = P;
    for (int d = 1; d < NCH; d <<= 1) {
      __syncthreads();
      float S2 = 0.f, P2 = 1.f;
      const bool has = (ch + d < NCH);
      if (has) {
        S2 = sS[(ch + d) * EB + el];
        P2 = sP[(ch + d) * EB + el];
      }
      __syncthreads();
      if (has) {
        S = S + P * S2;
        P = P * P2;
        sS[ch * EB + el] = S;
        sP[ch * EB + el] = P;
      }
    }
    __syncthreads();
    const float cin = carry[el];
    const float Ain = (ch + 1 < NCH) ? sS[(ch + 1) * EB + el] + sP[(ch + 1) * EB + el] * cin : cin;
    const float Afirst = sS[el] + sP[el] * cin;
    __syncthreads();
    if (ch == 0) carry[el] = Afirst;
    if (live) {
#pragma unroll
      for (int k = 0; k < LC; ++k) {
        const int t = t0 + k;
        if (t >= 0) {
          const size_t o = (size_t)t * E + e;
          const float A = a[k] + cp[k] * Ain;
          gae_st(adv + o, A);
          gae_st(ret + o, A + vv[k]);
        }
      }
    }
  }
}

template <int LC, int EB>
static hipError_t launch_scan(const float* rew, const float* val, const float* es, const float* lv, const float* dn,
                              float* adv, float* ret, int T, int E, float g, float gl, hipStream_t s, int max_chunks = 1024 / EB) {
  int NCH = (T + LC - 1) / LC;
  int maxch = max_chunks < 1024 / EB ? max_chunks : 1024 / EB;
  static int nch_env = -1;
  if (nch_env < 0) {
    const char* e = getenv("PH_GAE_NCH");
    nch_env = e ? atoi(e) : 0;
  }
  if (nch_env > 0 && nch_env < maxch) maxch = nch_env;
  if (NCH > maxch) NCH = maxch;
  dim3 grid((E + EB - 1) / EB), block(NCH * EB);
  const size_t lds = sizeof(float) * (2 * NCH * EB + EB);
  hipLaunchKernelGGL((gae_scan_kernel<LC, EB>), grid, block, lds, s, rew, val, es, lv, dn, adv, ret, T, E, NCH, g, gl);
  return hipGetLastError();
}

hipError_t launch_gae(const float* rew, const float* val, const float* es, const float* lv, const float* dn, float* adv,
                      float* ret, int T, int E, double gamma, double lam, int mode, hipStream_t s) {
  const float g = (float)gamma;
  const float gl = (float)(gamma * lam);
  if (mode == 0) mode = 2;
  if (mode == 1) {
    hipLaunchKernelGGL(gae_serial_kernel, dim3((E + 63) / 64), dim3(64), 0, s, rew, val, es, lv, dn, adv, ret, T, E, g,
                       gl);
    return hipGetLastError();
  }
  static int lc_env = -1;
  if (lc_env < 0) {
    const char* e = getenv("PH_GAE_LC");
    lc_env = e ? atoi(e) : 0;
  }
  if (lc_env == 8) return launch_scan<8, 32>(rew, val, es, lv, dn, adv, ret, T, E, g, gl, s);
  if (lc_env == 16) return launch_scan<16, 32>(rew, val, es, lv, dn, adv, ret, T, E, g, gl, s);
  if (lc_env == 32) return launch_scan<32, 32>(rew, val, es, lv, dn, adv, ret, T, E, g, gl, s);
  if (T <= 256) return launch_scan<8, 32>(rew, val, es, lv, dn, adv, ret, T, E, g, gl, s);
  if (E >= 16384) return launch_scan<16, 64>(rew, val, es, lv, dn, adv, ret, T, E, g, gl, s, 16);
  return launch_scan<16, 32>(rew, val, es, lv, dn, adv, ret, T, E, g, gl, s, 8);
}

__global__ void buffer_add_kernel(float* __restrict__ d_obs, float* __restrict__ d_act, float* __restrict__ d_rew,
                                  float* __restrict__ d_es, float* __restrict__ d_val, float* __restrict__ d_lp,
                                  const float* __restrict__ obs, const float* __restrict__ act,
                                  const float* __restrict__ es, const float* __restrict__ val,
                                  const float* __restrict__ lp, int E, int D, int A) {
  const int stride = gridDim.x * blockDim.x;
  const int g0 = blockIdx.x * blockDim.x + threadIdx.x;
  for (int i = g0; i < E * D; i += stride) d_obs[i] = obs[i];
  for (int i = g0; i < E * A; i += stride) d_act[i] = act[i];
  for (int i = g0; i < E; i += stride) {
    d_rew[i] = 0.f;
    d_es[i] = es[i];
    d_val[i] = val[i];
    d_lp[i] = lp[i];
  }
}
hipError_t launch_buffer_add(float* d_obs, float* d_act, float* d_rew, float* d_es, float* d_val, float* d_lp,
                             const float* obs, const float* act, const float* es, const float* val, const float* lp,
                             int E, int D, int A, hipStream_t s) {
  const int n = E * D;
  int blocks = (n + 255) / 256;
  if (blocks > 2048) blocks = 2048;
  if (blocks < 1) blocks = 1;
  hipLaunchKernelGGL(buffer_add_kernel, dim3(blocks), dim3(256), 0, s, d_obs, d_act, d_rew, d_es, d_val, d_lp, obs, act,
                     es, val, lp, E, D, A);
  return hipGetLastError();
}

struct CompactArgs {
  ph_rollout src, dst;
  const int* cols;
  int n, D, A;
};
__global__ void buffer_compact_kernel(CompactArgs a) {
  const int T = a.src.T, E = a.src.E, n = a.n;
  const size_t stride = (size_t)gridDim.x * blockDim.x, g0 = (size_t)blockIdx.x * blockDim.x + threadIdx.x;
  for (size_t i = g0; i < (size_t)T * n * a.D; i += stride) {
    const size_t row = i / a.D, f = i - row * a.D, t = row / n, c = row - t * n;
    a.dst.observations[i] = a.src.observations[(t * E + a.cols[c]) * a.D + f];
  }
  for (size_t i = g0; i < (size_t)T * n * a.A; i += stride) {
    const size_t row = i / a.A, f = i - row * a.A, t = row / n, c = row - t * n;
    a.dst.actions[i] = a.src.actions[(t * E + a.cols[c]) * a.A + f];
  }
  for (size_t i = g0; i < (size_t)T * n; i += stride) {
    const size_t t = i / n, c = i - t * n, j = t * E + a.cols[c];
    a.dst.rewards[i] = a.src.rewards[j];
    a.dst.episode_starts[i] = a.src.episode_starts[j];
    a.dst.values[i] = a.src.values[j];
    a.dst.log_probs[i] = a.src.log_probs[j];
    a.dst.advantages[i] = a.src.advantages[j];
    a.dst.returns[i] = a.src.returns[j];
  }
}
hipError_t launch_buffer_compact(const ph_rollout& src, const ph_rollout& dst, const int* cols, int n, int D, int A,
                                 hipStream_t s) {
  CompactArgs a;
  a.src = src;
  a.dst = dst;
  a.cols = cols;
  a.n = n;
  a.D = D;
  a.A = A;
  size_t work = (size_t)src.T * n * (D > 0 ? D : 1);
  int blocks = (int)((work + 255) / 256);
  if (blocks > 4096) blocks = 4096;
  if (blocks < 1) blocks = 1;
  hipLaunchKernelGGL(buffer_compact_kernel, dim3(blocks), dim3(256), 0, s, a);
  return hipGetLastError();
}

__global__ void reward_add_kernel(float* __restrict__ rew_row, const float* __restrict__ reward,
                                  const unsigned char* __restrict__ env_mask, int E) {
  const int e = blockIdx.x * blockDim.x + threadIdx.x;
  if (e >= E) return;
  if (env_mask && !env_mask[e]) return;
  rew_row[e] += reward[e];
}
hipError_t launch_reward_add(float* rew_row, const float* reward, const unsigned char* env_mask, int E, hipStream_t s) {
  hipLaunchKernelGGL(reward_add_kernel, dim3((E + 255) / 256), dim3(256), 0, s, rew_row, reward, env_mask, E);
  return hipGetLastError();
// ... 55 lines not shown
```

### pantheonrl_amd/csrc/ph_launch.h

```cpp
#pragma once
#include "ph_device.h"

namespace ph {

__host__ __device__ inline unsigned p2p_stamp32(unsigned long long epoch, int T, int t) {
  return (unsigned)(epoch * (unsigned long long)T + (unsigned long long)t + 1ull);
}

__device__ __forceinline__ void p2p_note_timeout(unsigned long long* error, int kind, int t, unsigned long long index,
                                                 unsigned long long want, unsigned long long seen) {
  if (atomicAdd(error, 1ull) == 0ull) {
    error[1] = (unsigned long long)(unsigned)kind | ((unsigned long long)(unsigned)(t & 0xffffff) << 8) | (index << 32);
    error[2] = want;
    error[3] = seen;
  }
}

__device__ __forceinline__ void poll_backoff(int& polls) {
  if (polls < 16) __builtin_amdgcn_s_sleep(2);
  else if (polls < 64) __builtin_amdgcn_s_sleep(16);
  else __builtin_amdgcn_s_sleep(127);
  ++polls;
}

hipError_t allow_dynamic_lds(const void* kernel, size_t bytes);
int device_cu_count();

struct FwdArgs {
  NetDims nd;
  const float* params;
  const float* obs;
  int n;
  const unsigned char* mask;
  const float* uniforms;
  const float* given_actions;
  uint64_t seed, counter;
  const unsigned long long* epoch;
  int deterministic;
  int* act_i32;
  float* act_f32;
  float* values;
  float* logp;
  float* entropy;
  float* logits;
  float* rb_obs;
  float* rb_act;
  float* rb_rew;
  float* rb_es;
  float* rb_val;
  float* rb_logp;
  const float* es_in;
  long long* prof;
  float* prev_rew;
  const float* pending_reward;
  const int* pos_env;
  const unsigned char* rec_mask;
  int rb_T;
  const int* joint;
  const unsigned long long* joint_ll;
  const unsigned long long* ll_epoch;
  int ll_T, ll_t;
  unsigned long long ll_timeout;
  unsigned long long* ll_error;
  int n_seats, seat;
  const int* partner_seat;
  float bonus;
  int reward_rule;
  const unsigned char* env_mask;
  unsigned int* host_done;
  unsigned int host_seq;
};

struct ScriptedSteps {
  int n_steps;
  const float* obs_seq;
  const float* rew_seq;
  const float* done_seq;
  const unsigned char* mask_seq;
  int mask_policy, mask_env;
};

constexpr int MAX_LOCAL_AGENTS = 4;
struct P2PStep {
  const ph_p2p* x;
  int t;
  int a_local;
  int persistent;
};
__host__ __device__ inline int p2p_persistent_slot(unsigned long long epoch, int T, int t) { return (int)(epoch & 1ull) * T + t; }
struct FwdMulti {
  FwdArgs a[MAX_LOCAL_AGENTS];
  P2PStep px;
};
struct ScriptedMulti {
  ScriptedSteps sc[MAX_LOCAL_AGENTS];
};
bool fwd16_eligible(const NetDims& nd, int n);
hipError_t launch_policy_fwd16_rollout(const FwdArgs& a, const ScriptedSteps& sc, int gemm_mode, hipStream_t s);
hipError_t launch_policy_fwd16_exchange_rollout(const FwdMulti& m, const ScriptedMulti& sm, int n_agents, hipStream_t s);
hipError_t exchange_rollout_blocks_per_cu(int* blocks_out);

struct GradArgs {
  NetDims nd;
  const float* params;
  const float* rb_obs;
  const float* rb_act;
  const float* rb_val;
  const float* rb_logp;
  const float* rb_adv;
  const float* rb_ret;
  int T, E;
  const int* idx;
  const int* idx_phys;
  uint32_t perm_n, perm_hb;
  uint64_t perm_seed;
  int perm_epoch;
  const unsigned long long* epoch;
  int mb_start;
  int nb;
  const float* advstats;
  float clip, clip_vf, ent_coef, vf_coef;
  int norm_adv;
  float* slabs;
  float* statpart;
  const int* stop_flag;
  long long* prof;
  int ntiles;
  const unsigned short* wimage;
  const uint4* ximg;
  int ximg_zero_row;
  const uint4* rec_pi;
  const uint4* rec_vf;
};

__device__ __host__ inline float joint_reward(int mine, int theirs, float bonus, int rule) {
  if (rule == 1) {
    const int d = (mine - theirs + 3) % 3;
    return d == 1 ? bonus : (d == 2 ? -bonus : 0.f);
  }
  return mine == theirs ? bonus : 0.f;
}

__device__ __host__ inline uint64_t epoch_key(uint64_t seed, int epoch) {
  uint64_t z = seed + 0x9E3779B97F4A7C15ull * (uint64_t)(epoch + 1);
  z = (z ^ (z >> 30)) * 0xBF58476D1CE4E5B9ull;
  z = (z ^ (z >> 27)) * 0x94D049BB133111EBull;
  return z ^ (z >> 31);
}

__device__ __forceinline__ int env_major_to_phys(int n, int T, int E) {
  const int e = n / T;
  return (n - e * T) * E + e;
}
__device__ __forceinline__ int minibatch_row(const GradArgs& a, int gi) {
  int n;
  if (a.idx) {
    n = a.idx[gi];
  } else {
    const uint64_t key = epoch_key(a.perm_seed + (a.epoch ? *a.epoch : 0ull), a.perm_epoch);
    n = (int)feistel_perm((uint32_t)(a.mb_start + gi), a.perm_n, a.perm_hb, key);
  }
  return env_major_to_phys(n, a.T, a.E);
}

struct alignas(16) AdamBias {
  float ss, bc2s;
  int step;
  int pad;
};

constexpr int ADV_SPLIT = 32;
constexpr int ADV_THREADS = 256;
struct AdvStatArgs {
  const float* rb_adv;
  int T, E;
  const int* perms;
  uint32_t perm_n, perm_hb;
  uint64_t perm_seed;
  const unsigned long long* epoch;
  int N, batch, n_mb;
  float* out;
  double* partial;
  int* idx_out;
  int* phys_out;
  uint4* rec_pi_out = nullptr;
  uint4* rec_vf_out = nullptr;
  const float *rb_logp = nullptr, *rb_act = nullptr, *rb_ret = nullptr, *rb_val = nullptr;
  const uint4* rowrec = nullptr;
  int* clear_flag = nullptr;
  AdamBias* adam_bias = nullptr;
  const int* opt_step = nullptr;
  float lr = 0.f, beta1 = 0.f, beta2 = 0.f;
};

struct ReduceArgs {
  const float* slabs;
  int nslab, P;
  int slab_len;
  const int* map;
  float* grad;
  float* blocksq;
  const float* statpart;
  int nstatpart;
  float* stats_out;
  int nb;
  float ent_coef, vf_coef, target_kl;
  int* stop_flag;
  int* step;
  float* scalars;
  const float* extra = nullptr;
  int n_extra = 0, extra_len = 0, extra_cut = 0, extra_lo = 0, extra_hi = 0;
  const float* extra_loss = nullptr;
  float extra_norm = 0.f;
  float extra_coef = 0.f;
  float* extra_loss_out = nullptr;
  int wide = 0;
};

struct AdamArgs {
  float* params;
  float* m;
  float* v;
  const float* grad;
  const float* blocksq;
  int nblk, P;
  const int* step;
  const float* scalars;
  int* stop_flag;
  float lr, beta1, beta2, eps, max_norm;
  float* stats_out;
  unsigned short* wimage;
  const int* wimage_map;
  const AdamBias* bias = nullptr;
};

struct StepArgs {
  ReduceArgs r;
  AdamArgs ad;
  unsigned long long* words = nullptr;
  unsigned int* gen = nullptr;
  unsigned long long timeout = 0;
  unsigned int* sweep_error = nullptr;
};

size_t fwd_lds_bytes(int R, int Lp);
size_t grad_lds_bytes(int R, int Lp, int onehot_D, int nchunk);
hipError_t launch_policy_fwd(const FwdArgs& a, int gemm_mode, hipStream_t s);
hipError_t launch_policy_fwd_multi(const FwdMulti& m, int n_agents, hipStream_t s);
hipError_t launch_fix_illegal(int* actions, const unsigned char* mask, int n, int L, hipStream_t s);
hipError_t launch_gae(const float* rew, const float* val, const float* es, const float* lv, const float* dn, float* adv,
                      float* ret, int T, int E, double gamma, double lam, int mode, hipStream_t s);
hipError_t launch_buffer_add(float* d_obs, float* d_act, float* d_rew, float* d_es, float* d_val, float* d_lp,
                             const float* obs, const float* act, const float* es, const float* val, const float* lp,
                             int E, int D, int A, hipStream_t s);
hipError_t launch_buffer_compact(const ph_rollout& src, const ph_rollout& dst, const int* cols, int n, int D, int A,
                                 hipStream_t s);
hipError_t launch_reward_add_ragged(float* rewards, const int* pos_env, const float* reward, const unsigned char* mask,
                                    int T, int E, hipStream_t s);
hipError_t launch_ragged_advance(int* pos_env, const unsigned char* mask, int T, int E, hipStream_t s);
hipError_t launch_liar_obs(const int* hands, const int* history, const int* nmoves, const unsigned char* is_ego,
                           const unsigned char* active, float* obs_out, int n, hipStream_t s);
hipError_t launch_liar_reset(int* hands, int* history, int* nmoves, const unsigned char* reset_mask,
                             unsigned char* ego_first, unsigned long long seed, unsigned long long counter,
                             const unsigned long long* epoch, float probegostart, int n, hipStream_t s);
hipError_t launch_reward_add(float* rew_row, const float* reward, const unsigned char* env_mask, int E, hipStream_t s);
hipError_t launch_reward_add_const(float* rew_row, float reward, int E, hipStream_t s);
hipError_t launch_reward_add_joint(float* rew_row, const float* base, const int* joint, int E, int n_seats, int seat,
                                   const int* partner_seat, float bonus, int rule, hipStream_t s);
hipError_t launch_framestack_push(float* stack, const float* obs, const unsigned char* reset_mask,
                                  const float* default_obs, int n, int D, int nf, hipStream_t s);
hipError_t launch_roundrobin_env_step(const int* joint, int* partnerid, const float* base, const float* done, float* reward_out,
                                      int* alt_action_out, float* next_block, int block_ld, int n_partners, float bonus, int n,
                                      hipStream_t s);
hipError_t launch_rps_step(const int* ego_act, const int* alt_act, float* ego_rew, float* alt_rew, int n, hipStream_t s);
hipError_t launch_liar_step(const int* hands, int* history, int* nmoves, const int* actions, const unsigned char* is_ego,
                            const unsigned char* active, float* obs_next, float* rew, unsigned char* done, int n,
                            hipStream_t s);
hipError_t launch_ppo_grad(const GradArgs& a, int nwg, int gemm_mode, hipStream_t s);
bool liar_rollout_eligible(const NetDims& nd, int n);

constexpr int ADAP_ROWS = 16;
struct AdapArgs {
  NetDims nd;
  const float* params;
  const float* rb_obs;
  int T, E;
  const int* idx;
  int nb;
  int ctx_size, n_ctx, n_states;
  int sampler;
  float coef;
  const int* state_idx;
  const float* contexts;
  uint64_t seed;
  const unsigned long long* epoch;
  uint32_t mbi, nb_hb;
  float* extra;
  float* loss_part;
  int* used_state_idx;
  float* used_contexts;
  const int* stop_flag;
  long long* prof;
};
struct AmWork {
  float *x, *xa, *y, *h;
  float *z, *v;
  float *dz, *dv;
  float *dzh, *dy, *dza;
  float *xg;
  float *act, *oldlp, *adv, *ret, *oldv;
};
struct AmGather {
  const float *rb_obs, *rb_act, *rb_logp, *rb_adv, *rb_ret, *rb_val;
  const int* idx;
  int nb, T, E, D, norm_adv;
  const float* advstats;
  float *xg, *act, *oldlp, *adv, *ret, *oldv;
};
struct AmCtx {
  const float* rb_obs;
  const int* idx;
  int nb, T, E, D;
  int ctx_size, n_ctx, n_states, sampler;
  const int* state_idx;
  const float* contexts;
  uint64_t seed;
  const unsigned long long* epoch;
  uint32_t mbi, nb_hb;
  float* rows;
  int* used_state_idx;
  float* used_contexts;
};
hipError_t am_forward_net(const ph_adapmult_layout& L, const float* params, int net, const float* X, int ldx, int rows,
                          const AmWork& w, hipStream_t s);
// ... 188 lines not shown
```

### pantheonrl_amd/csrc/ph_policy.hip

```cpp
#include <cstring>
#include <initializer_list>
#include "ph_rowtail.h"
#include "ph_liar_group.h"
#include "ph_pool.h"
#include "ph_bc_row.h"
#include "ph_adap_vec.h"

namespace ph {


constexpr int fwd_lds_floats(int R, int Lp) { return 2 * R * LDH + 2 * HID * LDH + (HID + R) * (Lp + 1) + 3 * 64 + R; }

template <int R, int NT>
struct AdapXStage {
  static constexpr int ITERS = R * HID / NT;
  int D, F, C, rows;
  const int* goff;
  const float* gobs;
  const float* gctx;
  int* off;
  float *obs, *ctx;
  __device__ __forceinline__ void stage(const int* rowphys, int tid) {
    constexpr int OD = 30, NO = (POOL_TILE * OD + NT - 1) / NT, NC = POOL_TILE * ADAP_VEC_MAX_CONTEXT / NT;
    float vo[NO], vc[NC];
    const int offv = tid <= OD ? goff[tid] : 0;
#pragma unroll
    for (int i = 0; i < NO; ++i) {
      const int e = tid + NT * i, r = e / OD;
      vo[i] = (r < rows) ? gobs[(size_t)rowphys[r] * OD + (e - r * OD)] : 0.f;
    }
#pragma unroll
    for (int i = 0; i < NC; ++i) {
      const int e = tid + NT * i, r = e / ADAP_VEC_MAX_CONTEXT, j = e % ADAP_VEC_MAX_CONTEXT;
      vc[i] = (r < rows && j < C) ? gctx[(size_t)rowphys[r] * C + j] : 0.f;
    }
    if (tid <= OD) off[tid] = offv;
#pragma unroll
    for (int i = 0; i < NO; ++i)
      if (tid + NT * i < POOL_TILE * OD) obs[tid + NT * i] = vo[i];
#pragma unroll
    for (int i = 0; i < NC; ++i) {
      const int e = tid + NT * i, r = e / ADAP_VEC_MAX_CONTEXT, j = e % ADAP_VEC_MAX_CONTEXT;
      if (j < C) ctx[r * C + j] = vc[i];
    }
  }
  __device__ __forceinline__ void issue(const int*, const float*, const NetDims&, int) {}
  __device__ __forceinline__ void commit(float* dst, const int*, const float*, const NetDims&, int c) const {
    const int tid = threadIdx.x, kk = tid & 63, f = c * HID + kk;
    AdapRowShape s;
    s.D = D;
    s.F = F;
    s.C = C;
    s.box = 0;
    float v[ITERS];
#pragma unroll
    for (int i = 0; i < ITERS; ++i) {
      const int r = (tid + NT * i) >> 6;
      v[i] = (r < rows && f < F + C) ? adap_row_value(s, off, obs + r * D, ctx + r * C, f) : 0.f;
    }
    __builtin_amdgcn_sched_barrier(0);
#pragma unroll
    for (int i = 0; i < ITERS; ++i) dst[((tid + NT * i) >> 6) * LDH + kk] = v[i];
  }
};

template <int R, int LP, bool VALU, class XS = XStage<R, R * 4>, bool MAP = false>
__device__ __forceinline__ void policy_fwd_body(const FwdArgs& a, XS xr = XS(), const int* map = nullptr, int rows = 0) {
  extern __shared__ __attribute__((aligned(16))) float smem[];
  constexpr int NT = R * 4;
  const NetDims& nd = a.nd;
  constexpr int Lp = LP, LDO = LP + 1;
  float* bufA = smem;
  float* bufB = bufA + R * LDH;
  float* w1s = bufB + R * LDH;
  float* w2s = w1s + HID * LDH;
  float* wos = w2s + HID * LDH;
  float* outs = wos + HID * LDO;
  float* b1s = outs + R * LDO;
  float* b2s = b1s + HID;
  float* bos = b2s + HID;
  int* rowphys = (int*)(bos + 64);

  const int tid = threadIdx.x;
  const int wave = tid >> 6, lane = tid & 63, li = lane & 31, lh = lane >> 5;
  const int mt = wave >> 1, nt = wave & 1;
  const int net = MAP ? 0 : blockIdx.y;
  const int row0 = blockIdx.x * R;
  const ph_layout& lay = nd.lay;
  const float* W1 = a.params + (net == 0 ? lay.pi_W1 : lay.vf_W1);
// ... 25 lines not shown
  xr.issue(rowphys, a.obs, nd, 0);
  w2r.commit(w2s);
  PH_STAMP(a.prof, 10);
  w1r.commit(w1s);
  if (net == 0) wor.commit(wos, Lp, LDO);
  if (tid < HID) {
    b1s[tid] = bias1;
    b2s[tid] = bias2;
    bos[tid] = bias3;
  }
  PH_STAMP(a.prof, 11);
  if constexpr (MAP) __syncthreads();
  xr.commit(bufA, rowphys, a.obs, nd, 0);
  __syncthreads();
  PH_STAMP(a.prof, 1);

  f32x16 acc = {0};
  for (int c = 0; c < nd.nchunk; ++c) {
    if (c > 0) {
      __syncthreads();
      w1r.issue(W1, c * HID, nd.F);
      xr.issue(rowphys, a.obs, nd, c);
      w1r.commit(w1s);
      xr.commit(bufA, rowphys, a.obs, nd, c);
      __syncthreads();
    }
    PH_STAMP(a.prof, 2);
    acc = tile_mma<false, false, VALU>(bufA, LDH, w1s, LDH, mt * 32, nt * 32, 0, HID, acc);
  }
  PH_STAMP(a.prof, 3);
#pragma unroll
  for (int r = 0; r < 16; ++r) {
    const int row = mt * 32 + drow(r, lh), col = nt * 32 + li;
    bufB[row * LDH + col] = fast_tanh(acc[r] + b1s[col]);
  }
  __syncthreads();
  PH_STAMP(a.prof, 4);

  f32x16 acc2 = {0};
  acc2 = tile_mma<false, false, VALU>(bufB, LDH, w2s, LDH, mt * 32, nt * 32, 0, HID, acc2);
#pragma unroll
  for (int r = 0; r < 16; ++r) {
    const int row = mt * 32 + drow(r, lh), col = nt * 32 + li;
    bufA[row * LDH + col] = fast_tanh(acc2[r] + b2s[col]);
  }
  __syncthreads();
  PH_STAMP(a.prof, 5);

  if (net == 1) {
    if (tid < R && rowphys[tid] >= 0) {
      float v = 0.f;
      for (int j = 0; j < HID; ++j) v = __builtin_fmaf(bufA[tid * LDH + j], bos[j], v);
      value_row_tail(a, row0 + tid, v + a.params[lay.val_b]);
    }
    copy_obs_rows(a, row0, (a.n - row0 < R) ? a.n - row0 : R, nd.D);
    PH_STAMP(a.prof, 7);
    return;
  }

  {
    const int ntn = Lp >> 5;
    if (wave < (R >> 5) * ntn) {
      const int hm = wave / ntn, hn = wave - hm * ntn;
      f32x16 acc3 = {0};
      acc3 = tile_mma<false, false, VALU>(bufA, LDH, wos, LDO, hm * 32, hn * 32, 0, HID, acc3);
#pragma unroll
      for (int r = 0; r < 16; ++r) {
        const int row = hm * 32 + drow(r, lh), col = hn * 32 + li;
        outs[row * LDO + col] = acc3[r] + bos[col];
      }
    }
  }
  __syncthreads();
  PH_STAMP(a.prof, 6);

  if (tid < R && rowphys[tid] >= 0) general_row_tail(a, nd, MAP ? rowphys[tid] : row0 + tid, outs + tid * LDO, fwd_counter(a));
  PH_STAMP(a.prof, 7);
}


__device__ __forceinline__ void lds_only_barrier() { asm volatile("s_waitcnt lgkmcnt(0)\n\ts_barrier" ::: "memory"); }
__device__ __forceinline__ void vm_drain() { __builtin_amdgcn_s_waitcnt(0x0F70); }

struct RowStage3 {
  static constexpr int ITERS = 6;
  static constexpr unsigned NONE = 0x80000000u;
  float v[ITERS] = {0.f, 0.f, 0.f, 0.f, 0.f, 0.f};
  __device__ __forceinline__ static unsigned base_offset(int row0, const NetDims& nd, int tid) {
    const int kk = tid & 63, w = (tid >> 6) - 1;
    return (w >= 0 && kk < nd.D && kk < nd.F) ? ((unsigned)(row0 + w) * (unsigned)nd.D + (unsigned)kk) * 4u : NONE;
  }
  __device__ __forceinline__ static unsigned slot_offset(unsigned base, int i, int D, int tid) {
    return (i == 5 && (tid >> 6) != 1) ? NONE : base + (unsigned)(3 * i) * (unsigned)D * 4u;
  }
  __device__ __forceinline__ static __amdgpu_buffer_rsrc_t block(const float* blk, int n, int D) {
    return __builtin_amdgcn_make_buffer_rsrc(const_cast<float*>(blk), 0, n * D * 4, 0x00020000);
  }
  __device__ __forceinline__ void issue(const float* obs, int n, const NetDims& nd, unsigned base, int tid) {
    const __amdgpu_buffer_rsrc_t rs = block(obs, n, nd.D);
#pragma unroll
    for (int i = 0; i < ITERS; ++i)
      v[i] = __builtin_bit_cast(float, __builtin_amdgcn_raw_buffer_load_b32(rs, slot_offset(base, i, nd.D, tid), 0, 0));
  }
  __device__ __forceinline__ void commit(float* dst, int tid) const {
    const int kk = tid & 63, w = (tid >> 6) - 1;
#pragma unroll
    for (int i = 0; i < ITERS; ++i) {
      const int r = w + 3 * i;
      if (r < 16) dst[r * LDH + kk] = v[i];
    }
  }
  __device__ __forceinline__ void copy_out(float* rb_obs, int n, int D, unsigned base, int tid) const {
    const __amdgpu_buffer_rsrc_t rs = block(rb_obs, n, D);
#pragma unroll
    for (int i = 0; i < ITERS; ++i)
      __builtin_amdgcn_raw_buffer_store_b32(__builtin_bit_cast(unsigned, v[i]), rs, slot_offset(base, i, D, tid), 0, 0);
  }
};

template <int CTRL>
__device__ __forceinline__ float dpp_quad_f(float v) {
  return __builtin_bit_cast(float, __builtin_amdgcn_update_dpp(0, __builtin_bit_cast(int, v), CTRL, 0xF, 0xF, true));
}
__device__ __forceinline__ float quad_sum_f(float v) {
  v += dpp_quad_f<0xB1>(v);
  v += dpp_quad_f<0x4E>(v);
  return v;
}

template <bool KEEP_JOINT>
__device__ __forceinline__ void fwd_args_pin_lean(FwdArgs& a) {
  a.mask = nullptr;
  a.uniforms = nullptr;
  a.given_actions = nullptr;
  a.deterministic = 0;
  a.act_f32 = nullptr;
  a.entropy = nullptr;
  a.logits = nullptr;
#ifndef PH_LEAN_PROF
  a.prof = nullptr;
#endif
  a.pos_env = nullptr;
  a.rec_mask = nullptr;
  if constexpr (!KEEP_JOINT) {
    a.joint = nullptr;
    a.joint_ll = nullptr;
  }
  a.env_mask = nullptr;
  a.host_done = nullptr;
  __builtin_assume(a.rb_obs != nullptr);
  __builtin_assume(a.rb_act != nullptr);
  __builtin_assume(a.rb_rew != nullptr);
  __builtin_assume(a.rb_es != nullptr);
  __builtin_assume(a.rb_val != nullptr);
  __builtin_assume(a.rb_logp != nullptr);
  __builtin_assume(a.es_in != nullptr);
}
bool fwd_args_lean(const FwdArgs& a, bool joint_ok = false) {
  static int enabled = -1;
  if (enabled < 0) {
    const char* e = getenv("PH_ROLLOUT_LEAN");
    enabled = (e && e[0] == '0') ? 0 : 1;
  }
#ifdef PH_LEAN_PROF
  constexpr bool lean_prof = true;
#else
  constexpr bool lean_prof = false;
#endif
  return enabled && !a.mask && !a.uniforms && !a.given_actions && !a.deterministic && !a.act_f32 && !a.entropy && !a.logits && (lean_prof || !a.prof) &&
         !a.pos_env && !a.rec_mask && (joint_ok || (!a.joint && !a.joint_ll)) && !a.env_mask && !a.host_done && a.rb_obs && a.rb_act && a.rb_rew &&
         a.rb_es && a.rb_val && a.rb_logp && a.es_in;
}

constexpr int ZS_FLOATS = 4 * 16 * 8;

struct TailWaveHook {
  bool arrive, alive;
  long long* stamp;
  __device__ __forceinline__ void split(int act, float lse) const {
    if (stamp) stamp[4] = (long long)clock64();
    if (arrive) asm volatile("s_waitcnt lgkmcnt(0)\n\ts_barrier" ::"v"(act), "v"(lse) : "memory");
    else asm volatile("" ::"v"(act), "v"(lse));
  }
  __device__ __forceinline__ bool live() const { return alive; }
};

template <bool VALU, int LEAN = 0, int TW = 0>
__device__ __forceinline__ void policy_fwd16_body(const FwdArgs& a0, const ph_p2p* px = nullptr, int px_t = 0, int px_a_local = 0,
                                                  int agent = 0, const ScriptedSteps* sc = nullptr, int px_persistent = 0) {
  extern __shared__ __attribute__((aligned(16))) float smem[];
  constexpr int R = 16, NT = 256;
  const NetDims& nd = a0.nd;
  FwdArgs a = a0;
  if constexpr (LEAN == 1) fwd_args_pin_lean<false>(a);
  if constexpr (LEAN == 2) fwd_args_pin_lean<true>(a);
  if constexpr (TW != 0) {
    a.mask = nullptr;
    a.env_mask = nullptr;
    a.uniforms = nullptr;
    a.given_actions = nullptr;
    a.deterministic = 0;
  }
#ifdef PH_LEAN_PROF
  long long* const prof0 = a0.prof;
#else
  long long* const prof0 = LEAN ? nullptr : a0.prof;
#endif
  float* xs = smem;
  float* hs = xs + R * LDH;
  float* zs = hs + R * LDH;
  int* rowphys = (int*)(zs + ZS_FLOATS);
  float* upre = (float*)(rowphys + 16);
  unsigned long long** pxll = (unsigned long long**)(upre + 32);

  const int tid = threadIdx.x;
  const int wave = TW ? __builtin_amdgcn_readfirstlane(tid >> 6) : tid >> 6, lane = tid & 63, c = lane & 15, g = lane >> 4;
  const bool lw = TW == 0 || wave < 4;
  const int net = blockIdx.y;
  const int row0 = blockIdx.x * R;
  const ph_layout& lay = nd.lay;
  const float* W1 = a.params + (net == 0 ? lay.pi_W1 : lay.vf_W1);
  const float* B1 = a.params + (net == 0 ? lay.pi_b1 : lay.vf_b1);
  const float* W2 = a.params + (net == 0 ? lay.pi_W2 : lay.vf_W2);
  const float* B2 = a.params + (net == 0 ? lay.pi_b2 : lay.vf_b2);
  const int nk = nd.L;

  PH_STAMP(a.prof, 0);
  if (tid < R) rowphys[tid] = (row0 + tid < a.n) ? row0 + tid : -1;
  constexpr bool PXH = LEAN != 0;
  const int pxw_h = (PXH && px) ? px->world : 0, pxc_h = (PXH && px) ? px->count : 0, pxr_h = (PXH && px) ? px->rank : 0;
  const int pxT_h = (PXH && px) ? px->T : 1, pxslots_h = (PXH && px) ? px->ll_slots : 1;
  unsigned long long* const ll_self_h = (PXH && px) ? px->ll[pxr_h] : nullptr;
  if (PXH && px && tid < pxw_h && tid < PH_MAX_RANKS) pxll[tid] = px->ll[tid];
#define pxw (PXH ? pxw_h : px->world)
#define pxc (PXH ? pxc_h : px->count)
#define pxr (PXH ? pxr_h : px->rank)
#define pxT (PXH ? pxT_h : px->T)
#define pxslots (PXH ? pxslots_h : px->ll_slots)
#define ll_self (PXH ? ll_self_h : px->ll[px->rank])
#define PXLL(p) (PXH ? pxll[p] : px->ll[p])
  float bw1[16], bw2[16], bwh[4];
  const int col = 16 * wave + c;
#pragma unroll
  for (int s = 0; s < 16; ++s) {
    const int k = g + 4 * s;
    bw1[s] = (lw && k < nd.F) ? W1[k * HID + col] : 0.f;
    bw2[s] = lw ? W2[k * HID + col] : 0.f;
  }
#pragma unroll
  for (int s = 0; s < 4; ++s) {
    const int k = g + 4 * (4 * wave + s);
    bwh[s] = 0.f;
    if (!lw) continue;
    if (net == 0) {
      if (c < nk) bwh[s] = a.params[lay.act_W + k * nk + c];
    } else if (c == 0) {
      bwh[s] = a.params[lay.val_W + k];
    }
  }
  const float bias1 = lw ? B1[col] : 0.f, bias2 = lw ? B2[col] : 0.f;
  float hbias = 0.f;
  if (wave == 0) {
    if (net == 0) hbias = (c < nk) ? a.params[lay.act_b + c] : 0.f;
    else hbias = (c == 0) ? a.params[lay.val_b] : 0.f;
  }
  XStage<R, NT> xr;
  lds_only_barrier();
  if (sc) a.obs = sc->obs_seq;
  const bool xsync = nd.obs_kind != PH_SPACE_BOX;
  if (lw) xr.issue(rowphys, a.obs, nd, 0);
  const bool staged = sc != nullptr && nd.obs_kind == PH_SPACE_BOX;
  const bool copy_staged = staged && net == 1 && a.rb_obs && !a.pos_env && (TW ? wave != 0 && wave < 4 : wave != 0);
  const unsigned roff = RowStage3::base_offset(row0, nd, tid);
  RowStage3 rows;
  if (copy_staged) rows.issue(a.obs, a0.n, nd, roff, tid);
  if (lw) xr.commit(xs, rowphys, a.obs, nd, 0);
  if (TW != 0 && !lw && xsync) lds_only_barrier();
  vm_drain();
  if (copy_staged) rows.copy_out(a.rb_obs, a0.n, nd.D, roff, tid);
  lds_only_barrier();
  PH_STAMP(a.prof, 1);

  const int n_steps = sc ? sc->n_steps : 1;
  unsigned long long epoch_hi = 0ull;
  if (sc) {
    epoch_hi = a0.epoch ? (unsigned long long)(*a0.epoch) << 32 : 0ull;
    a.epoch = nullptr;
    a.counter = a0.counter + epoch_hi;
  }
  const unsigned long long px_epoch = (px && px_persistent) ? *px->epoch : 0ull;
  const bool draw_ahead = sc && net == 0 && !a.uniforms && !a.deterministic && !a.given_actions;
  auto draw_uniforms = [&](int t1) {
    if (lane < R && row0 + lane < a0.n)
      upre[(t1 & 1) * R + lane] = philox_uniform(a0.seed, a0.counter + (unsigned long long)t1 + epoch_hi, (uint32_t)(row0 + lane), 0u);
  };
  if (TW == 0 && draw_ahead && wave == 1) draw_uniforms(0);

  auto product = [&](const float* A, const float (&bw)[16]) -> f32x4 {
    f32x4 e = {0.f, 0.f, 0.f, 0.f}, o = {0.f, 0.f, 0.f, 0.f};
    const float* ap = A + c * LDH + g;
    float av[16];
#pragma unroll
    for (int s = 0; s < 16; ++s) av[s] = ap[4 * s];
    __builtin_amdgcn_sched_barrier(0);
#pragma unroll
    for (int s = 0; s < 16; s += 2) {
      e = mma16<VALU>(av[s], bw[s], e, lane);
      o = mma16<VALU>(av[s + 1], bw[s + 1], o, lane);
    }
    return e + o;
  };

  auto step_record = [&](FwdArgs& a, int t) {
    const size_t row = (size_t)t * a0.n;
    a.obs = sc->obs_seq + row * nd.D;
    a.counter = a0.counter + (unsigned long long)t + epoch_hi;
    a.rb_obs = a0.rb_obs + row * nd.D;
    a.rb_act = a0.rb_act + row * nd.A;
    a.rb_rew = a0.rb_rew + row;
    a.rb_es = a0.rb_es + row;
    a.rb_val = a0.rb_val + row;
    a.rb_logp = a0.rb_logp + row;
    a.es_in = sc->done_seq + (row - a0.n);
    a.pending_reward = sc->rew_seq + (row - a0.n);
    a.prev_rew = a0.rb_rew + (row - a0.n);
    if constexpr (!LEAN && TW == 0) {
      a.mask = (sc->mask_seq && sc->mask_policy) ? sc->mask_seq + row * nd.L : nullptr;
      a.env_mask = (sc->mask_seq && sc->mask_env) ? sc->mask_seq + row * nd.L : nullptr;
    }
    if (px_persistent && a0.joint) {
      a.joint = a0.joint;
      a.joint_ll = ll_self + (size_t)p2p_persistent_slot(px_epoch, pxT, t - 1) * pxw * pxc;
      a.ll_t = t - 1;
    }
    a.prof = nullptr;
  };

  auto row_tail = [&](const FwdArgs& a, int t, int r, int grow, const ValuePre& vpre, const float* up, long long* pstep, auto hook) {
    float z[8];
    {
      float4 q[4][2];
#pragma unroll
      for (int w = 0; w < 4; ++w) {
        q[w][0] = *reinterpret_cast<const float4*>(zs + (w * R + r) * 8);
        q[w][1] = *reinterpret_cast<const float4*>(zs + (w * R + r) * 8 + 4);
      }
#pragma unroll
      for (int h = 0; h < 2; ++h) {
        z[4 * h + 0] = (q[0][h].x + q[1][h].x) + (q[2][h].x + q[3][h].x);
        z[4 * h + 1] = (q[0][h].y + q[1][h].y) + (q[2][h].y + q[3][h].y);
        z[4 * h + 2] = (q[0][h].z + q[1][h].z) + (q[2][h].z + q[3][h].z);
        z[4 * h + 3] = (q[0][h].w + q[1][h].w) + (q[2][h].w + q[3][h].w);
      }
    }
    if (net == 0) {
      const uint64_t ctr = fwd_counter(a);
      int act;
      switch (nk) {
        case 1: act = discrete8_row_tail<1>(a, nd, grow, z, ctr, up, pstep, hook); break;
        case 2: act = discrete8_row_tail<2>(a, nd, grow, z, ctr, up, pstep, hook); break;
        case 3: act = discrete8_row_tail<3>(a, nd, grow, z, ctr, up, pstep, hook); break;
        case 4: act = discrete8_row_tail<4>(a, nd, grow, z, ctr, up, pstep, hook); break;
        case 5: act = discrete8_row_tail<5>(a, nd, grow, z, ctr, up, pstep, hook); break;
        case 6: act = discrete8_row_tail<6>(a, nd, grow, z, ctr, up, pstep, hook); break;
        case 7: act = discrete8_row_tail<7>(a, nd, grow, z, ctr, up, pstep, hook); break;
        default: act = discrete8_row_tail<8>(a, nd, grow, z, ctr, up, pstep, hook); break;
      }
      if (px && hook.live()) {
        const int pt = px_t + t;
        const int slot = px_persistent ? p2p_persistent_slot(px_epoch, pxT, pt) : pt % pxslots;
        const size_t off = (size_t)slot * pxw * pxc + (size_t)(pxr * px_a_local + agent) * a.n + grow;
        const unsigned long long w =
            ((unsigned long long)p2p_stamp32(px_persistent ? px_epoch : *px->epoch, pxT, pt) << 32) | (unsigned long long)(unsigned)act;
        for (int p = 0; p < pxw; ++p)
          __hip_atomic_store(PXLL(p) + off, w, __ATOMIC_RELAXED, __HIP_MEMORY_SCOPE_SYSTEM);
      }
    } else {
      if (hook.live()) {
        value_row_tail(a, grow, z[0], !a.pos_env && a.rb_val, vpre);
        if (sc && t == n_steps - 1) {
          float add = sc->rew_seq[(size_t)t * a0.n + grow];
          if (px_persistent && a0.joint) {
            FwdArgs b = a;
            b.joint_ll = ll_self + (size_t)p2p_persistent_slot(px_epoch, pxT, t) * pxw * pxc;
            b.ll_t = t;
            int p = *a0.partner_seat;
            p = p < 0 ? 0 : (p >= a0.n_seats ? a0.n_seats - 1 : p);
            const int mine = ll_read(b, b.joint_ll + (size_t)a0.seat * a0.n + grow);
            const int theirs = ll_read(b, b.joint_ll + (size_t)p * a0.n + grow);
            add += joint_reward(mine, theirs, a0.bonus, a0.reward_rule);
          }
          a.rb_rew[grow] += add;
        }
      }
      hook.split(0, z[0]);
    }
  };

  if constexpr (TW != 0) {
    if (!lw) {
      const int nlive = (a0.n - row0 < R) ? a0.n - row0 : R;
      const int r = lane < nlive ? lane : nlive - 1, grow = row0 + r;
      const bool live = lane < nlive;
#ifdef PH_LEAN_PROF
      long long* const wstamp = (prof0 && lane == 0) ? prof0 + ((size_t)blockIdx.y * gridDim.x + blockIdx.x) * 16 : nullptr;
#else
      long long* const wstamp = nullptr;
#endif
      auto draw = [&](int t) { return philox_uniform(a0.seed, a0.counter + (unsigned long long)t + epoch_hi, (uint32_t)grow, 0u); };
      auto preload = [&](const FwdArgs& a) {
        return (net == 1 && !a.pos_env && a.rb_val) ? value_row_preload(a, grow) : ValuePre{0.f, 0.f, 0.f, 0ull, 0ull, 0u, 0, 0};
      };
      if (draw_ahead) upre[r] = draw(0);
      ValuePre vpre = preload(a);
      lds_only_barrier();
      lds_only_barrier();
      lds_only_barrier();
      for (int s = 0; s < n_steps; ++s) {
        const bool more = s + 1 < n_steps;
        if (more) {
          if (xsync) lds_only_barrier();
          lds_only_barrier();
        }
        long long* const ws = (s == 7) ? wstamp : nullptr;
        if (ws) ws[2] = (long long)clock64();
        row_tail(a, s, r, grow, vpre, draw_ahead ? upre + r : nullptr, nullptr, TailWaveHook{more, live, ws});
        if (ws) ws[6] = (long long)clock64();
        if (more) {
          step_record(a, s + 1);
          vpre = preload(a);
          lds_only_barrier();
          if (draw_ahead) upre[r] = draw(s + 1);
          lds_only_barrier();
        }
      }
      return;
    }
    __builtin_amdgcn_s_setprio(1);
  }

  for (int t = 0; t < n_steps; ++t) {
  long long* const pstep = (sc && t == 8) ? prof0 : nullptr;
  PH_STAMP(pstep, 8);
  if (t > 0) {
    step_record(a, t);
    if (!staged) {
      xr.issue(rowphys, a.obs, nd, 0);
      xr.commit(xs, rowphys, a.obs, nd, 0);
      vm_drain();
    }
    lds_only_barrier();
  }
  PH_STAMP(pstep, 9);
  const bool more = t + 1 < n_steps;
  const float* const obs_next = sc ? sc->obs_seq + (size_t)(t + 1) * a0.n * nd.D : nullptr;
  if (TW != 0 && staged && more && wave != 0) rows.issue(obs_next, a0.n, nd, roff, tid);

  const bool pre_ok = TW == 0 && net == 1 && wave == 0 && lane < R && row0 + lane < a.n && !a.pos_env && a.rb_val;
  ValuePre vpre = {0.f, 0.f, 0.f, 0ull, 0ull, 0u, 0, 0};
  if (pre_ok) vpre = value_row_preload(a, row0 + lane);
  const bool copy_from_regs = net == 1 && a.rb_obs && !a.pos_env && nd.obs_kind == PH_SPACE_BOX;
  {
    const f32x4 z1 = product(xs, bw1);
#pragma unroll
    for (int r = 0; r < 4; ++r) hs[(4 * g + r) * LDH + col] = fast_tanh(z1[r] + bias1);
  }
  lds_only_barrier();
  PH_STAMP(a.prof, 3);
  PH_STAMP(pstep, 10);
  {
    const f32x4 z2 = product(hs, bw2);
#pragma unroll
    for (int r = 0; r < 4; ++r) xs[(4 * g + r) * LDH + col] = fast_tanh(z2[r] + bias2);
  }
  lds_only_barrier();
  PH_STAMP(a.prof, 5);
  PH_STAMP(pstep, 11);

  if (TW == 0 && staged && net == 1 && more && wave != 0) rows.issue(obs_next, a0.n, nd, roff, tid);

  {
    if (wave == 0 && pre_ok) value_row_preload_words(a, row0 + lane, vpre);
    const float* ap = xs + c * LDH + g + 16 * wave;
    float av[4];
#pragma unroll
    for (int j = 0; j < 4; ++j) av[j] = ap[4 * j];
    f32x4 e = {0.f, 0.f, 0.f, 0.f}, o = {0.f, 0.f, 0.f, 0.f};
    e = mma16<VALU>(av[0], bwh[0], e, lane);
    o = mma16<VALU>(av[1], bwh[1], o, lane);
    e = mma16<VALU>(av[2], bwh[2], e, lane);
    o = mma16<VALU>(av[3], bwh[3], o, lane);
    const f32x4 zh = e + o;
    if (c < 8) {
#pragma unroll
      for (int r = 0; r < 4; ++r) zs[(wave * R + 4 * g + r) * 8 + c] = zh[r] + hbias;
    }
  }
  lds_only_barrier();
  PH_STAMP(pstep, 12);
  if (sc) vm_drain();
  if (staged && more && wave != 0 && lw) {
    if (net == 1 || TW != 0) {
      rows.commit(xs, tid);
      if (copy_staged) rows.copy_out(a0.rb_obs + (size_t)(t + 1) * a0.n * nd.D, a0.n, nd.D, roff, tid);
    }
  }
  if (TW != 0) PH_STAMP(pstep, 13);
  if (TW == 0 && wave == 0) {
    PH_STAMP(pstep, 13);
    const int r = lane, grow = row0 + lane;
    if (r < R && grow < a.n) row_tail(a, t, r, grow, vpre, draw_ahead ? upre + (t & 1) * R + r : nullptr, pstep, TailNoHook{});
  }
  PH_STAMP(pstep, 14);
  const bool stage_here = TW == 0 && staged && net == 0 && more && wave != 0;
  if (stage_here) rows.issue(obs_next, a0.n, nd, roff, tid);
  if (TW == 0 && draw_ahead && wave == 1 && more) draw_uniforms(t + 1);
  if (stage_here) {
    rows.commit(xs, tid);
    vm_drain();
  }
  if (copy_from_regs) {
    if (!staged) {
      const int kk = tid & 63;
#pragma unroll
      for (int i = 0; i < XStage<R, NT>::ITERS; ++i) {
        const int rr = (tid + NT * i) >> 6;
        if (kk < nd.D && row0 + rr < a.n) a.rb_obs[(size_t)(row0 + rr) * nd.D + kk] = xr.v[i];
      }
    }
  } else if (net == 1) {
    copy_obs_rows(a, row0, (a.n - row0 < R) ? a.n - row0 : R, nd.D, TW ? tid : -1, NT);
  }
  PH_STAMP(a.prof, 7);
  PH_STAMP(pstep, 15);
  }
}

#undef pxw
#undef pxc
#undef pxr
#undef pxT
#undef pxslots
#undef ll_self
#undef PXLL

template <bool VALU, bool LEAN = false>
__global__ __launch_bounds__(256) void policy_fwd16_kernel(FwdArgs a) {
  policy_fwd16_body<VALU, LEAN ? 1 : 0>(a);
  if constexpr (!LEAN) {
    if (a.host_done) {
      __threadfence_system();
      __syncthreads();
      if (threadIdx.x == 0) __hip_atomic_store(a.host_done + blockIdx.y, a.host_seq, __ATOMIC_RELEASE, __HIP_MEMORY_SCOPE_SYSTEM);
    }
  }
}
constexpr int ROLLOUT_THREADS = 320;
template <bool VALU, bool LEAN>
__global__ __launch_bounds__(VALU ? 256 : ROLLOUT_THREADS) void policy_fwd16_rollout_kernel(FwdArgs a, ScriptedSteps sc) {
  policy_fwd16_body<VALU, LEAN ? 1 : 0, VALU ? 0 : 4>(a, nullptr, 0, 0, 0, &sc);
}
template <bool LEAN>
__global__ __launch_bounds__(256) void policy_fwd16_multi_kernel(FwdMulti m) {
  policy_fwd16_body<false, LEAN ? 2 : 0>(m.a[blockIdx.z], m.px.x, m.px.t, m.px.a_local, blockIdx.z);
}
template <bool LEAN>
__global__ __launch_bounds__(256, 3) void policy_fwd16_exchange_rollout_kernel(FwdMulti m, ScriptedMulti sm) {
  policy_fwd16_body<false, LEAN ? 2 : 0>(m.a[blockIdx.z], m.px.x, 0, m.px.a_local, blockIdx.z, &sm.sc[blockIdx.z], 1);
}

static size_t fwd16_lds_bytes() { return sizeof(float) * (size_t)(2 * 16 * LDH + ZS_FLOATS + 16 + 32) + sizeof(void*) * PH_MAX_RANKS; }

bool fwd16_eligible(const NetDims& nd, int n) {
  static int enabled = -1;
  if (enabled < 0) {
    const char* e = getenv("PH_FWD16");
    enabled = (e && e[0] == '0') ? 0 : 1;
  }
  return enabled && !nd.gauss && nd.nchunk == 1 && nd.A == 1 && nd.L <= 8 && n < 16384;
}

template <bool VALU>
static hipError_t launch_fwd16_variant(const FwdArgs& a, hipStream_t s) {
  const size_t lds = fwd16_lds_bytes();
  const bool general = VALU || !fwd_args_lean(a);
  const void* fn = general ? (const void*)policy_fwd16_kernel<VALU> : (const void*)policy_fwd16_kernel<false, true>;
  if (const hipError_t e = allow_dynamic_lds(fn, lds); e != hipSuccess) return e;
// ... 1172 lines not shown
```

### pantheonrl_amd/csrc/ph_ppo.hip

```cpp
#include "ph_launch.h"
#include "ph_ppo_loss.h"
#include "ph_split.h"
#include "ph_step.h"

namespace ph {


template <int N>
__device__ __forceinline__ float lds_colsum(const float* p, int stride, float s) {
#pragma unroll
  for (int r0 = 0; r0 < N; r0 += 16) {
    float t[16];
#pragma unroll
    for (int i = 0; i < 16; ++i) t[i] = p[(r0 + i) * stride];
    __builtin_amdgcn_sched_barrier(0);
#pragma unroll
    for (int i = 0; i < 16; ++i) s += t[i];
  }
  return s;
}
template <int N>
__device__ __forceinline__ float lds_coldot(const float* p, int stride, const float* q, int qstride, float s) {
#pragma unroll
  for (int r0 = 0; r0 < N; r0 += 16) {
// ... 634 lines not shown
  *ntiles = (nb + 63) / 64;
  *nwg = *ntiles < num_cu ? *ntiles : num_cu;
  if (nd.split == 2 && *nwg > num_cu / 2 && num_cu >= 2) *nwg = num_cu / 2;
}

hipError_t launch_ppo_grad(const GradArgs& a, int nwg, int gemm_mode, hipStream_t s) {
  if (a.nd.split == 2) return launch_ppo_grad_split_oh(a, nwg, s);
  if (a.nd.split) return launch_ppo_grad_split(a, nwg, s);
  if (grad_fast_eligible(a.nd)) return launch_ppo_grad_fast(a, nwg, gemm_mode, s);
  if (a.nd.Lp != 32 && a.nd.Lp != 64) return hipErrorInvalidValue;
  const bool lp64 = a.nd.Lp == 64;
  if (gemm_mode == 1) return lp64 ? launch_grad_shape<64, true>(a, nwg, s) : launch_grad_shape<32, true>(a, nwg, s);
  return lp64 ? launch_grad_shape<64, false>(a, nwg, s) : launch_grad_shape<32, false>(a, nwg, s);
}

__device__ __forceinline__ void st_rec(uint4* p, const uint4& v) {
  typedef unsigned int u32x4_t __attribute__((ext_vector_type(4)));
  __builtin_nontemporal_store((u32x4_t){v.x, v.y, v.z, v.w}, reinterpret_cast<u32x4_t*>(p));
}
__global__ __launch_bounds__(ADV_THREADS) void adv_stats_kernel(AdvStatArgs a) {
  __shared__ double sh[2][ADV_THREADS / 64];
  const int mb = blockIdx.x / ADV_SPLIT, seg = blockIdx.x - mb * ADV_SPLIT;
  const int ep = mb / a.n_mb, k = mb - ep * a.n_mb;
  const int start = k * a.batch;
  const int nb = (a.N - start < a.batch) ? a.N - start : a.batch;
  const uint64_t key = epoch_key(a.perm_seed + (a.epoch ? *a.epoch : 0ull), ep);
  const int tid = threadIdx.x, lane = tid & 63, wave = tid >> 6;
  if (a.clear_flag && blockIdx.x == 0 && tid == 0) *a.clear_flag = 0;
  const int chunk = (nb + ADV_SPLIT - 1) / ADV_SPLIT;
  const int lo = seg * chunk, hi = (lo + chunk < nb) ? lo + chunk : nb;
  auto value = [&](int i) -> double {
    if (i >= hi) return 0.0;
    int n;
    if (a.perms) {
      n = a.perms[(size_t)ep * a.N + start + i];
    } else {
      n = (int)feistel_perm((uint32_t)(start + i), a.perm_n, a.perm_hb, key);
      if (a.idx_out) a.idx_out[(size_t)ep * a.N + start + i] = n;
    }
    const int phys = env_major_to_phys(n, a.T, a.E);
    if (a.phys_out) a.phys_out[(size_t)ep * a.N + start + i] = phys;
    float adv;
    if (a.rec_pi_out && a.rowrec) {
      const uint4 rp = a.rowrec[2 * (size_t)phys], rv = a.rowrec[2 * (size_t)phys + 1];
      const size_t o = (size_t)ep * a.N + start + i;
      adv = __uint_as_float(rp.x);
      st_rec(a.rec_pi_out + o, make_uint4((unsigned)phys, rp.x, rp.y, rp.z));
      st_rec(a.rec_vf_out + o, make_uint4((unsigned)phys, rv.x, rv.y, 0u));
    } else {
      adv = a.rb_adv[phys];
      if (a.rec_pi_out) {
        const size_t o = (size_t)ep * a.N + start + i;
        st_rec(a.rec_pi_out + o, make_uint4((unsigned)phys, __float_as_uint(adv), __float_as_uint(a.rb_logp[phys]), __float_as_uint(a.rb_act[phys])));
        st_rec(a.rec_vf_out + o, make_uint4((unsigned)phys, __float_as_uint(a.rb_ret[phys]), __float_as_uint(a.rb_val[phys]), 0u));
      }
    }
    return (double)adv;
  };
  double s = 0.0, q = 0.0;
  for (int i = lo + tid; i < hi; i += 4 * ADV_THREADS) {
    const double v0 = value(i), v1 = value(i + ADV_THREADS), v2 = value(i + 2 * ADV_THREADS), v3 = value(i + 3 * ADV_THREADS);
    s += (v0 + v1) + (v2 + v3);
    q += (v0 * v0 + v1 * v1) + (v2 * v2 + v3 * v3);
  }
  for (int off = 32; off > 0; off >>= 1) {
    s += __shfl_down(s, off, 64);
    q += __shfl_down(q, off, 64);
  }
  if (lane == 0) {
    sh[0][wave] = s;
    sh[1][wave] = q;
  }
  __syncthreads();
  if (tid == 0) {
    double ts = 0.0, tq = 0.0;
    for (int w = 0; w < ADV_THREADS / 64; ++w) {
      ts += sh[0][w];
      tq += sh[1][w];
    }
    a.partial[((size_t)mb * ADV_SPLIT + seg) * 2 + 0] = ts;
    a.partial[((size_t)mb * ADV_SPLIT + seg) * 2 + 1] = tq;
  }
}
__global__ void adv_finalize_kernel(AdvStatArgs a, int n_total) {
  const int mb = blockIdx.x * blockDim.x + threadIdx.x;
  if (mb >= n_total) return;
  if (a.adam_bias) {
    AdamBias b;
    b.step = *a.opt_step + 1 + mb;
    b.pad = 0;
    adam_step_scalars(b.step, a.lr, a.beta1, a.beta2, &b.ss, &b.bc2s);
    a.adam_bias[mb] = b;
  }
  const int k = mb % a.n_mb;
  const int start = k * a.batch;
  const int nb = (a.N - start < a.batch) ? a.N - start : a.batch;
  double ts = 0.0, tq = 0.0;
  for (int seg = 0; seg < ADV_SPLIT; ++seg) {
    ts += a.partial[((size_t)mb * ADV_SPLIT + seg) * 2 + 0];
    tq += a.partial[((size_t)mb * ADV_SPLIT + seg) * 2 + 1];
  }
  const double mean = ts / (double)nb;
  double var = (nb > 1) ? (tq - (double)nb * mean * mean) / (double)(nb - 1) : 0.0;
  if (var < 0.0) var = 0.0;
  a.out[2 * mb + 0] = (float)mean;
  a.out[2 * mb + 1] = (float)sqrt(var);
}
hipError_t launch_adv_stats(const AdvStatArgs& a, int n_total, hipStream_t s) {
  hipLaunchKernelGGL(adv_stats_kernel, dim3(n_total * ADV_SPLIT), dim3(ADV_THREADS), 0, s, a);
  hipLaunchKernelGGL(adv_finalize_kernel, dim3((n_total + 63) / 64), dim3(64), 0, s, a, n_total);
  return hipGetLastError();
}

constexpr int OP_ROWS = 32;
struct RowScalars {
  const float *adv, *logp, *act, *ret, *val;
  uint4* rowrec;
};
__global__ __launch_bounds__(256) void obs_planes_kernel(const float* __restrict__ obs, int n, int D, int F, int fold,
                                                         uint4* __restrict__ image, RowScalars rs) {
  __shared__ float xs[OP_ROWS][65];
  const int tid = threadIdx.x;
  const size_t row0 = (size_t)blockIdx.x * OP_ROWS;
  const int nrow = (row0 + OP_ROWS <= (size_t)n) ? OP_ROWS : (int)((size_t)n > row0 ? (size_t)n - row0 : 0);
  const float* src = obs + row0 * D;
  for (int e = tid; e < nrow * D; e += 256) {
    const int r = e / D, f = e - r * D;
    if (f < F) xs[r][f] = __builtin_nontemporal_load(src + e);
  }
  __syncthreads();
  const int r = tid >> 3, g = tid & 7;
  const size_t row = row0 + r;
  if (row > (size_t)n) return;
  if (rs.rowrec && row < (size_t)n && g < 2) {
    uint4 v = make_uint4(0u, 0u, 0u, 0u);
    if (g == 0) v = make_uint4(__float_as_uint(rs.adv[row]), __float_as_uint(rs.logp[row]), __float_as_uint(rs.act[row]), 0u);
    else v = make_uint4(__float_as_uint(rs.ret[row]), __float_as_uint(rs.val[row]), 0u, 0u);
    rs.rowrec[2 * row + g] = v;
  }
  typedef __bf16 bf8 __attribute__((ext_vector_type(8)));
  bf8 pl[3];
#pragma unroll
  for (int e = 0; e < 8; ++e) {
    const int f = 8 * g + e;
    float x = 0.f;
    if (row < (size_t)n) x = f < F ? xs[r][f] : ((fold && f == HID - 1) ? 1.f : 0.f);
    __bf16 h, m, l;
    split1(x, h, m, l);
    pl[0][e] = h;
    pl[1][e] = m;
    pl[2][e] = l;
  }
#pragma unroll
  for (int p = 0; p < 3; ++p) image[row * XIMG_ROW_U4 + p * 8 + g] = __builtin_bit_cast(uint4, pl[p]);
}
hipError_t launch_obs_planes(const float* obs, int n, int D, int F, int fold, uint4* image, const float* adv, const float* logp,
                             const float* act, const float* ret, const float* val, uint4* rowrec, hipStream_t s) {
  const size_t blocks = ((size_t)n + 1 + OP_ROWS - 1) / OP_ROWS;
  RowScalars rs{adv, logp, act, ret, val, (adv && logp && act && ret && val) ? rowrec : nullptr};
  hipLaunchKernelGGL(obs_planes_kernel, dim3((unsigned)blocks), dim3(256), 0, s, obs, n, D, F, fold, image, rs);
  return hipGetLastError();
}

template <int VEC>
__global__ __launch_bounds__(RED_PARAMS * 4) void ppo_reduce_kernel(ReduceArgs a) {
  __shared__ float lds_union[4 * RED_PARAMS];
  static_assert(4 * RED_PARAMS >= 32 * NSTATP + NSTATP || 4 * RED_PARAMS >= 32 * NSTATP, "statistics scratch within the slab scratch");
  float (*gsum)[RED_PARAMS] = reinterpret_cast<float (*)[RED_PARAMS]>(lds_union);
  float (*part)[NSTATP] = reinterpret_cast<float (*)[NSTATP]>(lds_union);
  __shared__ float means[NSTATP];
  const int tid = threadIdx.x;
  const int stop_word = uniform_word(a.stop_flag);
  if (blockIdx.x == gridDim.x - 1) {
    if (__builtin_amdgcn_readfirstlane(stop_word) == 0) (void)reduce_statistics(a, part, means, true);
    return;
  }
  const int fetched = reduce_dst_fetch(a, blockIdx.x);
  reduce_quarters<VEC>(a, gsum, blockIdx.x);
  if (__builtin_amdgcn_readfirstlane(stop_word) != 0) {
    if (blockIdx.x == 0) step_stopped(a);
    return;
  }
  const int dst = reduce_dst_select(a, blockIdx.x, fetched);
  const float g = reduce_fold(a, gsum, dst);
  if (tid < 64) {
    if (dst >= 0) a.grad[dst] = g;
    float q = g * g;
    for (int off = 32; off > 0; off >>= 1) q += __shfl_down(q, off, 64);
    if (tid == 0) a.blocksq[blockIdx.x] = q;
  }
}

template <int VEC>
// ... 167 lines not shown
```

### pantheonrl_amd/vec.py

```python
from __future__ import annotations

import ctypes as C
from typing import Optional

import numpy as np
import torch as th

from . import _native as nat
from .ppo import PPO, require_mlp_kernels


class VecOnPolicyAgent:

    def __init__(self, model: PPO):
        self.model = model
        pol, rb = model.policy, model.rollout_buffer
        self._require_kernels(pol)
        E, lay, dev = rb.n_envs, pol.layout, pol.device
        self.E = E
        self._last_episode_starts = th.ones(E, dtype=th.float32, device=dev)
        self.n_steps = 0
        self.num_timesteps = 0
        self.iteration = 0
        self.actions = th.zeros((E, lay.A), dtype=th.int32, device=dev)
        self.values = th.zeros((E,), dtype=th.float32, device=dev)
        self.log_probs = th.zeros((E,), dtype=th.float32, device=dev)
        self._lib, self._h = pol.ctx.lib, pol.ctx.handle
        self._rb = C.byref(rb.c_struct())
        self.sync_stats = False
        self._pending = None
        self.episode_stats = None

    def _require_kernels(self, pol) -> None:
        require_mlp_kernels(pol, type(self).__name__)

    def get_action(self, obs: th.Tensor, record: bool = True, action_mask: Optional[th.Tensor] = None,
                   episode_start: Optional[th.Tensor] = None) -> th.Tensor:
        model = self.model
        pol, rb = model.policy, model.rollout_buffer
        if record and self.n_steps >= model.n_steps:
            self.learn_from_buffer()
        es = self._last_episode_starts if episode_start is None else episode_start
        pending = self._pending if (record and rb.pos >= 1) else None
        pol._counter += 1
        nat.check(pol._native_forward(
            pol.params.data_ptr(), obs.data_ptr(), self.E, nat.ptr(action_mask), None, None,
            pol._seed, pol._counter, 0, self.actions.data_ptr(), None, self.values.data_ptr(),
            self.log_probs.data_ptr(), None, None, self._rb if record else None, rb.pos if record else 0,
            es.data_ptr() if record else None, nat.ptr(pending), int(pol.gemm_mode)))
        if pending is not None:
            self._pending = None
        if record:
            rb.pos += 1
            rb.full = rb.pos == rb.buffer_size
        self.n_steps += 1
        self.num_timesteps += self.E
        return self.actions

    def rollout_scripted(self, data: "SyntheticRollouts") -> None:
        model = self.model
        pol, rb = model.policy, model.rollout_buffer
        if rb.pos != 0 or data.T != rb.buffer_size or data.E != self.E:
            raise nat.NativeError("rollout_scripted: needs an empty rollout buffer of data.T rows and data.E environments")
        self.flush_rewards()
        nat.check(pol._native_scripted(
            pol.params.data_ptr(), data.obs.data_ptr(), data.rewards.data_ptr(), data.dones.data_ptr(),
            self.E, data.T, self._last_episode_starts.data_ptr(), pol._seed, pol._counter + 1, self.actions.data_ptr(),
            self.values.data_ptr(), self.log_probs.data_ptr(), self._rb, 0, int(pol.gemm_mode)))
        pol._counter += data.T
        rb.pos, rb.full = data.T, True
        self.n_steps += data.T
        self.num_timesteps += data.T * self.E
        self._last_episode_starts = data.dones[data.T - 1]
        self._pending = None

    def update(self, reward: th.Tensor, done: th.Tensor, env_mask: Optional[th.Tensor] = None) -> None:
        if self._pending is not None or env_mask is not None:
            self.flush_rewards()
        if env_mask is None:
            self._pending = reward
        else:
            rb = self.model.rollout_buffer
            nat.check(self._lib.ph_buffer_add_reward(self._h, self._rb, rb.pos - 1, reward.data_ptr(),
                                                     nat.ptr(env_mask)))
        self._last_episode_starts = done

    def update_joint(self, base_reward: th.Tensor, done: th.Tensor, joint: th.Tensor, seat: int,
                     partner_seat: th.Tensor, bonus: float = 0.01) -> None:
        self.flush_rewards()
        rb = self.model.rollout_buffer
        nat.check(self._lib.ph_buffer_add_reward_joint(self._h, self._rb, rb.pos - 1, base_reward.data_ptr(),
                                                       joint.data_ptr(), int(joint.shape[0]), int(seat),
                                                       partner_seat.data_ptr(), float(bonus)))
        self._last_episode_starts = done

    def flush_rewards(self) -> None:
        if self._pending is not None:
            rb = self.model.rollout_buffer
            nat.check(self._lib.ph_buffer_add_reward(self._h, self._rb, rb.pos - 1, self._pending.data_ptr(), None))
            self._pending = None

    def compute_returns(self) -> None:
        rb = self.model.rollout_buffer
        self.flush_rewards()
        if self.episode_stats is not None:
            self.episode_stats.scan()
        nat.check(self._lib.ph_gae(self._h, self._rb, self.values.data_ptr(), self._last_episode_starts.data_ptr(),
                                   rb.gamma, rb.gae_lambda, int(rb.gae_mode)))

    def finish_update(self) -> None:
        rb = self.model.rollout_buffer
        self.iteration += 1
        rb.pos, rb.full = 0, False
        self.n_steps = 0

    def learn_from_buffer(self) -> None:
        self.compute_returns()
        self.model.train(sync_stats=self.sync_stats)
        self.finish_update()

    def bind_stream(self) -> None:
        self.model.policy._bind()


def require_tower_lds(pol, who: str) -> None:
    try:
        nat.require_arch_fits(pol.spec, pol.arch)
    except nat.NativeError as exc:
        raise nat.NativeError(f"{who}: {exc}") from None


def is_tower(pol) -> bool:
    from .ppo import ArchActorCriticPolicy
    return isinstance(pol, ArchActorCriticPolicy)


class TowerVecOnPolicyAgent(VecOnPolicyAgent):

    def _require_kernels(self, pol) -> None:
        if not is_tower(pol):
            raise nat.NativeError(f"{type(self).__name__}: {type(pol).__name__} is not a net_arch tower policy; use VecOnPolicyAgent")
        require_tower_lds(pol, type(self).__name__)


def is_adap(pol) -> bool:
    from .adap import AdapPolicy, AdapPolicyMult
    return isinstance(pol, AdapPolicy) and not isinstance(pol, AdapPolicyMult)
# ... 39 lines not shown
        nat.check(self._lib.ph_adap_context_draw(self._h, self.sampler, self.context_size, pol._seed, int(counter), nat.ptr(flags),
                                                 self.contexts.data_ptr(), self.E))

    def _paid_done(self, flags: th.Tensor) -> None:
        if self.latent_syncer is None:
            counter = self.model.policy._counter if self.draw_counter is None else self.draw_counter
            self.redraw(flags.to(th.uint8).contiguous(), counter)


class AdapVecOnPolicyAgent(AdapSeat, VecOnPolicyAgent):

    def __init__(self, model: PPO, latent_syncer: Optional[AdapSeat] = None):
        super().__init__(model)
        self._init_adap(latent_syncer)

    def get_action(self, obs: th.Tensor, record: bool = True, action_mask: Optional[th.Tensor] = None,
                   episode_start: Optional[th.Tensor] = None) -> th.Tensor:
        if record and self.n_steps >= self.model.n_steps:
            self.learn_from_buffer()
        return super().get_action(self.build_rows(obs), record, action_mask, episode_start)

    def update(self, reward: th.Tensor, done: th.Tensor, env_mask: Optional[th.Tensor] = None) -> None:
        super().update(reward, done, env_mask)
        self._paid_done((done != 0) if env_mask is None else ((done != 0) & env_mask.bool()))

    def rollout_scripted(self, data) -> None:
        raise nat.NativeError("AdapVecOnPolicyAgent.rollout_scripted: the one-launch scripted rollout does not build ADAP rows or "
                              "redraw contexts; step with get_action / update")


def vec_agent_for(model: PPO, latent_syncer=None) -> VecOnPolicyAgent:
    if is_adap(model.policy):
        return AdapVecOnPolicyAgent(model, latent_syncer)
    return (TowerVecOnPolicyAgent if is_tower(model.policy) else VecOnPolicyAgent)(model)


class VecFrameStack:

    def __init__(self, n_envs: int, obs_dim: int, numframes: int, ctx: nat.Context, device, default_obs=None):
        self.E, self.D, self.nf, self.ctx, self.device = n_envs, obs_dim, numframes, ctx, device
        self.default = None if default_obs is None else th.as_tensor(
            np.asarray(default_obs, np.float32)).to(device).contiguous()
        self.stack = th.zeros((n_envs, numframes * obs_dim), dtype=th.float32, device=device)
        if self.default is not None:
            self.stack.copy_(self.default.repeat(numframes).expand(n_envs, -1))

    def push(self, obs: th.Tensor, reset_mask: Optional[th.Tensor] = None) -> th.Tensor:
        self.ctx.set_stream(th.cuda.current_stream(self.device).cuda_stream)
        nat.check(self.ctx.lib.ph_framestack_push(self.ctx.handle, self.stack.data_ptr(), obs.data_ptr(),
                                                  nat.ptr(reset_mask), nat.ptr(self.default), self.E, self.D, self.nf))
        return self.stack


class SyntheticRollouts:

    def __init__(self, observation_space, n_envs: int, n_steps: int, horizon: int, seed: int, device):
        rng = np.random.default_rng(seed)
        T, E = n_steps, n_envs
        kind = type(observation_space).__name__
        if kind == "Box":
            D = int(np.prod(observation_space.shape))
            obs = rng.standard_normal((T, E, D), dtype=np.float32)
        elif kind == "Discrete":
            obs = rng.integers(0, observation_space.n, size=(T, E, 1)).astype(np.float32)
        else:
            nvec = np.asarray(observation_space.nvec)
            obs = (rng.random((T, E, len(nvec))) * nvec).astype(np.int64).astype(np.float32)
        self.obs = th.as_tensor(obs).to(device)
        self.rewards = th.as_tensor(rng.standard_normal((T, E), dtype=np.float32)).to(device)
        self.dones = th.as_tensor((rng.random((T, E)) < 1.0 / max(horizon, 1)).astype(np.float32)).to(device)
        self.T, self.E = T, E


class RPSTables:

    def __init__(self, n_envs: int, n_steps: int, device):
        T, E = n_steps, n_envs
        self.obs = th.zeros((T, E, 1), dtype=th.float32, device=device)
        self.rewards = th.zeros((T, E), dtype=th.float32, device=device)
        self.dones = th.ones((T, E), dtype=th.float32, device=device)
        self.T, self.E = T, E


def run_iteration_eager(agent: VecOnPolicyAgent, data: SyntheticRollouts, scripted: bool = False) -> None:
    agent.bind_stream()
    if scripted:
        agent.rollout_scripted(data)
    else:
        for t in range(data.T):
            agent.get_action(data.obs[t])
            agent.update(data.rewards[t], data.dones[t])
    agent.learn_from_buffer()


class IterationGraph:

    def __init__(self, agent: VecOnPolicyAgent, data: SyntheticRollouts, stream: th.cuda.Stream, scripted: bool = False):
        self.agent, self.data, self.stream, self.scripted = agent, data, stream, scripted
        pol = agent.model.policy
        self.epoch_word = th.zeros(1, dtype=th.int64, device=pol.device)
        nat.check(pol.ctx.lib.ph_ctx_set_rng_epoch(pol.ctx.handle, self.epoch_word.data_ptr()))
        agent.model.device_permutations = True
        with th.cuda.stream(stream):
            run_iteration_eager(agent, data, scripted)
            run_iteration_eager(agent, data, scripted)
            stream.synchronize()
            agent.bind_stream()
            lib, h = pol.ctx.lib, pol.ctx.handle
            nat.check(lib.ph_graph_begin(h))
            try:
                run_iteration_eager(agent, data, scripted)
                nat.check(lib.ph_rng_epoch_advance(h))
            finally:
                gid = C.c_int(-1)
                nat.check(lib.ph_graph_end(h, C.byref(gid)))
            self.graph_id = gid.value

    def launch(self) -> None:
        pol = self.agent.model.policy
        nat.check(pol.ctx.lib.ph_graph_launch(pol.ctx.handle, self.graph_id))
        self.agent.iteration += 1
        self.agent.num_timesteps += self.data.T * self.data.E


def run_joint_iteration_eager(agents, datas, streams) -> None:
    for agent, data, stream in zip(agents, datas, streams):
        with th.cuda.stream(stream):
            agent.bind_stream()
            for t in range(data.T):
                agent.get_action(data.obs[t])
                agent.update(data.rewards[t], data.dones[t])
            agent.compute_returns()
    PPO.train_joint([agent.model for agent in agents])
    for agent in agents:
        agent.finish_update()


class JointIterationGraph:

    def __init__(self, agents, datas, streams):
        self.agents, self.datas, self.streams = list(agents), list(datas), list(streams)
        lead = self.agents[0].model.policy
        self.epoch_words = []
        for agent in self.agents:
            pol = agent.model.policy
            word = th.zeros(1, dtype=th.int64, device=pol.device)
            nat.check(pol.ctx.lib.ph_ctx_set_rng_epoch(pol.ctx.handle, word.data_ptr()))
            self.epoch_words.append(word)
            agent.model.device_permutations = True
        s0, others = self.streams[0], self.streams[1:]
        fork, joins = th.cuda.Event(), [th.cuda.Event() for _ in others]
        for _ in range(2):
            run_joint_iteration_eager(self.agents, self.datas, self.streams)
            fork.record(s0)
            for s, j in zip(others, joins):
                s.wait_event(fork)
                j.record(s)
                s0.wait_event(j)
        th.cuda.synchronize(lead.device)
        with th.cuda.stream(s0):
            self.agents[0].bind_stream()
        lib, h = lead.ctx.lib, lead.ctx.handle
        nat.check(lib.ph_graph_begin(h))
        try:
            fork.record(s0)
            for s in others:
                s.wait_event(fork)
            run_joint_iteration_eager(self.agents, self.datas, self.streams)
            for agent in self.agents:
                pol = agent.model.policy
                nat.check(pol.ctx.lib.ph_rng_epoch_advance(pol.ctx.handle))
            for s, j in zip(others, joins):
                j.record(s)
                s0.wait_event(j)
        finally:
            gid = C.c_int(-1)
            nat.check(lib.ph_graph_end(h, C.byref(gid)))
        self.graph_id = gid.value
        self._lib, self._h = lib, h

    def launch(self) -> None:
        nat.check(self._lib.ph_graph_launch(self._h, self.graph_id))
        for agent, data in zip(self.agents, self.datas):
            agent.iteration += 1
            agent.num_timesteps += data.T * data.E


class FusedSelfPlayRollout:

    def __init__(self, agents, datas, exchange, stream: th.cuda.Stream, bonus: float = 0.01, update_graphs: bool = True,
                 masks=None, mask_mode: int = 2, persistent: Optional[bool] = None, reward_rule: str = "match"):
        self.agents, self.datas, self.exchange, self.stream, self.bonus = agents, datas, exchange, stream, bonus
        for a in agents:
            require_mlp_kernels(a.model.policy, type(self).__name__)
# ... 159 lines not shown
```

Before: 127.2 million agent-steps/s.

## Build PPO grad pack ahead during rollout and GAE, fold weight image into finalize

The scripted rollout kernel now writes the split-precision observation image for the gradient kernel as it stages each step. GAE writes the per-row records (advantage, return, value, log-prob, action) directly, so train_prepare can skip the separate obs_planes pack kernel. The weight-image rebuild kernel is merged into the advantage-finalize kernel as extra blocks, removing one launch. The aim is to drop whole-buffer re-reads and kernel launches per iteration, at the cost of extra stores in the rollout and GAE kernels plus stage-tracking state that must stay consistent across graph capture.

```diff
diff --git a/include/pantheon_hip.h b/include/pantheon_hip.h
--- a/include/pantheon_hip.h
+++ b/include/pantheon_hip.h
@@ -156,6 +156,11 @@
 
 int ph_gae(ph_ctx *ctx, const ph_rollout *rb, const float *last_values , const float *dones ,
            double gamma, double gae_lambda, int mode);
+
+int ph_grad_pack_arm(ph_ctx *ctx, int on);
+int ph_debug_grad_pack_copy(ph_ctx *ctx, void *ximg_out, size_t ximg_u4, void *rowrec_out, size_t rowrec_u4);
+int ph_debug_grad_pack_build(ph_ctx *ctx, const ph_spec *spec, const ph_rollout *rb, void *ximg_out, void *rowrec_out);
+int ph_debug_grad_pack_stage(ph_ctx *ctx, int *stage_out );
 
 int ph_policy_forward(ph_ctx *ctx, const ph_spec *spec, const float *params, const float *obs, int n,
                       const unsigned char *action_mask, const float *uniforms, const float *given_actions,
diff --git a/pantheonrl_amd/_native.py b/pantheonrl_amd/_native.py
--- a/pantheonrl_amd/_native.py
+++ b/pantheonrl_amd/_native.py
@@ -297,6 +297,10 @@
     "ph_buffer_add_reward_joint": [_vp, C.POINTER(PhRollout), _i, _vp, _vp, _i, _i, _vp, C.c_float],
     "ph_buffer_reset": [_vp, C.POINTER(PhSpec), C.POINTER(PhRollout)],
     "ph_gae": [_vp, C.POINTER(PhRollout), _vp, _vp, _d, _d, _i],
+    "ph_grad_pack_arm": [_vp, _i],
+    "ph_debug_grad_pack_copy": [_vp, _vp, C.c_size_t, _vp, C.c_size_t],
+    "ph_debug_grad_pack_build": [_vp, C.POINTER(PhSpec), C.POINTER(PhRollout), _vp, _vp],
+    "ph_debug_grad_pack_stage": [_vp, C.POINTER(_i)],
     "ph_policy_forward": [_vp, C.POINTER(PhSpec), _vp, _vp, _i, _vp, _vp, _vp, _ull, _ull, _i, _vp, _vp, _vp, _vp, _vp,
                           _vp, C.POINTER(PhRollout), _i, _vp, _vp, _i],
     "ph_ctx_set_joint_reward_rule": [_vp, _i],
diff --git a/pantheonrl_amd/csrc/ph_abi.hip b/pantheonrl_amd/csrc/ph_abi.hip
--- a/pantheonrl_amd/csrc/ph_abi.hip
+++ b/pantheonrl_amd/csrc/ph_abi.hip
@@ -144,6 +144,11 @@
   size_t rec_cap = 0;
   uint4* rowrec = nullptr;
   size_t rowrec_cap = 0;
+  bool pack_armed = false;
+  int pack_stage = 0;
+  const float* pack_obs = nullptr;
+  int pack_T = 0, pack_E = 0, pack_spec = 0;
+  long long ximg_zero_rows = -1;
   unsigned long long* step_words = nullptr;
   size_t step_words_cap = 0;
   unsigned int* step_gen = nullptr;
@@ -463,6 +468,7 @@
   fwd_eval_fields(a, action_mask, uniforms, given_actions, deterministic, actions_f32, entropy, logits);
   a.prof = ctx->prof;
   if (fwd_bind_row(who, a, rb, pos, episode_start_in, pending_reward)) return 1;
+  if (rb) ctx->pack_stage = 0;
   if (arch) {
     PH_HIP(ph::launch_arch_fwd(a, ad, gemm_mode, ctx->stream));
     return 0;
@@ -488,9 +494,13 @@
   a.prof = ctx->prof;
   a.deterministic = deterministic;
   fwd_bind_bases(a, rb, episode_start_in, pos_env, record_mask);
+  ctx->pack_stage = 0;
   PH_HIP(arch ? ph::launch_arch_fwd(a, ad, gemm_mode, ctx->stream) : ph::launch_policy_fwd(a, gemm_mode, ctx->stream));
   return 0;
 }
+
+int pack_ahead_rollout(ph_ctx* ctx, const ph::NetDims& fwd_nd, const ph_rollout* rb, int pos0, int n_steps, int gemm_mode,
+                       ph::ScriptedSteps* sc);
 
 int scripted_rollout_run(const char* who, ph_ctx* ctx, const ph_spec* spec, const ph_arch* arch, const float* params,
                          const float* obs_seq, const float* rew_seq, const float* done_seq, int n, int n_steps,
@@ -517,6 +527,10 @@
   sc.obs_seq = obs_seq;
   sc.rew_seq = rew_seq;
   sc.done_seq = done_seq;
+  ctx->pack_stage = 0;
+  const bool armed = ctx->pack_armed;
+  ctx->pack_armed = false;
+  if (armed && !arch && pack_ahead_rollout(ctx, a.nd, rb, pos0, n_steps, gemm_mode, &sc)) return 1;
   PH_HIP(arch ? ph::launch_arch_rollout(a, ad, sc, gemm_mode, ctx->stream)
               : ph::launch_policy_fwd16_rollout(a, sc, gemm_mode, ctx->stream));
   return 0;
@@ -1133,8 +1147,18 @@
   if (check_rb(rb)) return 1;
   if (!last_values || !dones) return fail("ph_gae: null last_values/dones");
   if (mode < 0 || mode > 2) return fail("ph_gae: mode must be 0, 1 or 2");
+  const bool rec = ctx->pack_stage == 1 && ctx->pack_obs == rb->observations && ctx->pack_T == rb->T && ctx->pack_E == rb->E &&
+                   ctx->rowrec && ctx->rowrec_cap >= 2 * (size_t)rb->T * rb->E;
+  ctx->pack_stage = rec ? 2 : 0;
   PH_HIP(ph::launch_gae(rb->rewards, rb->values, rb->episode_starts, last_values, dones, rb->advantages, rb->returns,
-                        rb->T, rb->E, gamma, gae_lambda, mode, ctx->stream));
+                        rb->T, rb->E, gamma, gae_lambda, mode, ctx->stream, rec ? ctx->rowrec : nullptr, rb->log_probs, rb->actions));
+  return 0;
+}
+
+int ph_grad_pack_arm(ph_ctx* ctx, int on) {
+  if (!ctx) return fail("null ctx");
+  ctx->pack_armed = on != 0;
+  ctx->pack_stage = 0;
   return 0;
 }
 
@@ -2579,7 +2603,7 @@
   g.rec_vf = ctx->rec_vf;
 }
 
-int rebuild_weight_image(ph_ctx* ctx, const ph::NetDims& nd, const float* params) {
+int rebuild_weight_image(ph_ctx* ctx, const ph::NetDims& nd, const float* params, bool launch = true) {
   if (!nd.split) return 0;
   if ((size_t)nd.wimage_elems > ctx->wimage_cap) {
     if (ctx->capturing) return fail("first split-kernel use inside graph capture: call it once outside capture first");
@@ -2591,24 +2615,57 @@
     PH_HIP(hipMemsetAsync(ctx->wimage, 0, (size_t)nd.wimage_elems * sizeof(unsigned short), ctx->stream));
     ctx->wimage_zeroed_for = nd.spec_id;
   }
-  PH_HIP(ph::launch_weight_image(params, ctx->wimage, nd.wimage_map, nd.lay.P, ctx->stream));
-  return 0;
-}
-
-int build_grad_pack(ph_ctx* ctx, const ph::NetDims& nd, const ph_rollout* rb, size_t n_rec) {
+  if (launch) PH_HIP(ph::launch_weight_image(params, ctx->wimage, nd.wimage_map, nd.lay.P, ctx->stream));
+  return 0;
+}
+
+void select_gemm(ph::NetDims& nd, int gemm_mode);
+int ensure_grad_pack_rows(ph_ctx* ctx, size_t rows) {
+  const size_t need_img = (rows + 1) * ph::XIMG_ROW_U4;
+  if (need_img > ctx->ximg_cap) ctx->ximg_zero_rows = -1;
+  if (ensure(ctx, ctx->ximg, ctx->ximg_cap, need_img)) return 1;
+  return ensure(ctx, ctx->rowrec, ctx->rowrec_cap, 2 * rows);
+}
+int pack_ahead_rollout(ph_ctx* ctx, const ph::NetDims& fwd_nd, const ph_rollout* rb, int pos0, int n_steps, int gemm_mode,
+                       ph::ScriptedSteps* sc) {
+  ph::NetDims nd = fwd_nd;
+  select_gemm(nd, gemm_mode);
+  if (nd.split != 1 || nd.obs_kind != PH_SPACE_BOX || pos0 != 0 || n_steps != rb->T) return 0;
+  const size_t rows = (size_t)rb->T * rb->E;
+  const bool ready = (rows + 1) * ph::XIMG_ROW_U4 <= ctx->ximg_cap && 2 * rows <= ctx->rowrec_cap && ctx->ximg_zero_rows == (long long)rows;
+  if (!ready) {
+    if (ctx->capturing) return 0;
+    if (ensure_grad_pack_rows(ctx, rows)) return 1;
+    PH_HIP(hipMemsetAsync(ctx->ximg + rows * ph::XIMG_ROW_U4, 0, ph::XIMG_ROW_U4 * sizeof(uint4), ctx->stream));
+    ctx->ximg_zero_rows = (long long)rows;
+  }
+  sc->ximg = ctx->ximg;
+  sc->ximg_fold = ph::grad_fast_fold(nd) ? 1 : 0;
+  ctx->pack_stage = 1;
+  ctx->pack_obs = rb->observations;
+  ctx->pack_T = rb->T;
+  ctx->pack_E = rb->E;
+  ctx->pack_spec = nd.spec_id;
+  return 0;
+}
+
+int build_grad_pack(ph_ctx* ctx, const ph::NetDims& nd, const ph_rollout* rb, size_t n_rec, bool may_be_ahead = false) {
+  const bool ahead = may_be_ahead && nd.split == 1 && ctx->pack_stage == 2 && ctx->pack_obs == rb->observations && ctx->pack_T == rb->T &&
+                     ctx->pack_E == rb->E && ctx->pack_spec == nd.spec_id;
+  ctx->pack_stage = 0;
   if (nd.split != 1) return 0;
   const size_t rows = (size_t)rb->T * rb->E;
-  const size_t need_img = (rows + 1) * ph::XIMG_ROW_U4;
-  if (ensure(ctx, ctx->ximg, ctx->ximg_cap, need_img)) return 1;
-  if (ensure(ctx, ctx->rowrec, ctx->rowrec_cap, 2 * rows)) return 1;
+  if (ensure_grad_pack_rows(ctx, rows)) return 1;
   if (n_rec > ctx->rec_cap) {
     size_t c1 = ctx->rec_cap, c2 = ctx->rec_cap;
     if (ensure(ctx, ctx->rec_pi, c1, n_rec)) return 1;
     if (ensure(ctx, ctx->rec_vf, c2, n_rec)) return 1;
     ctx->rec_cap = n_rec;
   }
+  if (ahead) return 0;
   PH_HIP(ph::launch_obs_planes(rb->observations, (int)rows, nd.D, nd.F, ph::grad_fast_fold(nd) ? 1 : 0, ctx->ximg, rb->advantages,
                                rb->log_probs, rb->actions, rb->returns, rb->values, ctx->rowrec, ctx->stream));
+  ctx->ximg_zero_rows = (long long)rows;
   return 0;
 }
 void fill_adv_records(ph::AdvStatArgs& aa, const ph_ctx* ctx, const ph::NetDims& nd, const ph_rollout* rb) {
@@ -2751,6 +2808,12 @@
   aa.lr = t.hp->learning_rate;
   aa.beta1 = t.hp->adam_beta1;
   aa.beta2 = t.hp->adam_beta2;
+  if (t.nd.split) {
+    aa.wi_image = t.ctx->wimage;
+    aa.wi_params = t.opt->params;
+    aa.wi_map = t.nd.wimage_map;
+    aa.wi_P = t.nd.lay.P;
+  }
 }
 
 int train_prepare(const char* who, TrainPlan& t, ph_ctx* ctx, const ph_spec* spec, const ph_opt_state* opt, const ph_rollout* rb,
@@ -2782,8 +2845,8 @@
                       (size_t)n_epochs * t.N))
     return 1;
   hipStream_t s = ctx->stream;
-  if (rebuild_weight_image(ctx, t.nd, opt->params)) return 1;
-  if (build_grad_pack(ctx, t.nd, rb, (size_t)n_epochs * t.N)) return 1;
+  if (rebuild_weight_image(ctx, t.nd, opt->params, false)) return 1;
+  if (build_grad_pack(ctx, t.nd, rb, (size_t)n_epochs * t.N, true)) return 1;
   t.hb = ph::feistel_half_bits((uint32_t)t.N);
   ph::AdvStatArgs aa;
   train_adv_args(t, need_idx, aa);
@@ -2877,6 +2940,35 @@
                  unsigned long long perm_seed, float* stats, int gemm_mode) {
   DevGuard dev_guard(ctx);
   return train_run("ph_ppo_train", ctx, spec, opt, rb, hp, n_epochs, batch_size, perms, perm_seed, stats, gemm_mode, nullptr);
+}
+
+int ph_debug_grad_pack_copy(ph_ctx* ctx, void* ximg_out, size_t ximg_u4, void* rowrec_out, size_t rowrec_u4) {
+  DevGuard dev_guard(ctx);
+  if (!ctx || !ximg_out || !rowrec_out) return fail("ph_debug_grad_pack_copy: null argument");
+  if (!ctx->ximg || !ctx->rowrec || ximg_u4 > ctx->ximg_cap || rowrec_u4 > ctx->rowrec_cap)
+    return fail("ph_debug_grad_pack_copy: the context holds no pack of that size");
+  PH_HIP(hipMemcpyAsync(ximg_out, ctx->ximg, ximg_u4 * sizeof(uint4), hipMemcpyDeviceToDevice, ctx->stream));
+  PH_HIP(hipMemcpyAsync(rowrec_out, ctx->rowrec, rowrec_u4 * sizeof(uint4), hipMemcpyDeviceToDevice, ctx->stream));
+  return 0;
+}
+
+int ph_debug_grad_pack_stage(ph_ctx* ctx, int* stage_out) {
+  if (!ctx || !stage_out) return fail("ph_debug_grad_pack_stage: null argument");
+  *stage_out = ctx->pack_stage;
+  return 0;
+}
+
+int ph_debug_grad_pack_build(ph_ctx* ctx, const ph_spec* spec, const ph_rollout* rb, void* ximg_out, void* rowrec_out) {
+  DevGuard dev_guard(ctx);
+  if (!ctx || !ximg_out || !rowrec_out) return fail("ph_debug_grad_pack_build: null argument");
+  if (check_rb(rb)) return 1;
+  ph::NetDims nd;
+  if (resolve(ctx, spec, &nd)) return 1;
+  select_gemm(nd, 2);
+  if (nd.split != 1) return fail("ph_debug_grad_pack_build: not a spec of ppo_grad_split_kernel");
+  PH_HIP(ph::launch_obs_planes(rb->observations, rb->T * rb->E, nd.D, nd.F, ph::grad_fast_fold(nd) ? 1 : 0, (uint4*)ximg_out,
+                               rb->advantages, rb->log_probs, rb->actions, rb->returns, rb->values, (uint4*)rowrec_out, ctx->stream));
+  return 0;
 }
 
 int ph_adap_train(ph_ctx* ctx, const ph_spec* spec, const ph_opt_state* opt, const ph_rollout* rb,
diff --git a/pantheonrl_amd/csrc/ph_gae.hip b/pantheonrl_amd/csrc/ph_gae.hip
--- a/pantheonrl_amd/csrc/ph_gae.hip
+++ b/pantheonrl_amd/csrc/ph_gae.hip
@@ -1,11 +1,22 @@
 #include "ph_launch.h"
 
 namespace ph {
+
+struct RowRecOut {
+  uint4* rowrec;
+  const float *logp, *act;
+  __device__ __forceinline__ void put(size_t o, float adv, float ret, float val, float lp, float ac) const {
+    rowrec[2 * o] = make_uint4(__float_as_uint(adv), __float_as_uint(lp), __float_as_uint(ac), 0u);
+    rowrec[2 * o + 1] = make_uint4(__float_as_uint(ret), __float_as_uint(val), 0u, 0u);
+  }
+  __device__ __forceinline__ void put(size_t o, float adv, float ret, float val) const { put(o, adv, ret, val, logp[o], act[o]); }
+};
 
 __global__ __launch_bounds__(64) void gae_serial_kernel(const float* __restrict__ rew, const float* __restrict__ val,
                                                         const float* __restrict__ es, const float* __restrict__ last_values,
                                                         const float* __restrict__ dones, float* __restrict__ adv,
-                                                        float* __restrict__ ret, int T, int E, float g, float gl) {
+                                                        float* __restrict__ ret, int T, int E, float g, float gl,
+                                                        RowRecOut rr) {
 #pragma clang fp contract(off)
   const int e = blockIdx.x * blockDim.x + threadIdx.x;
   if (e >= E) return;
@@ -29,6 +40,7 @@
       last = delta + ((gl * nnt) * last);
       adv[o] = last;
       ret[o] = last + v[u];
+      if (rr.rowrec) rr.put(o, last, last + v[u], v[u]);
       nv = v[u];
       nnt = 1.0f - s[u];
     }
@@ -40,6 +52,7 @@
     last = delta + ((gl * nnt) * last);
     adv[o] = last;
     ret[o] = last + v;
+    if (rr.rowrec) rr.put(o, last, last + v, v);
     nv = v;
     nnt = 1.0f - s;
   }
@@ -48,13 +61,13 @@
 __device__ __forceinline__ float gae_ld(const float* p) { return __builtin_nontemporal_load(p); }
 __device__ __forceinline__ void gae_st(float* p, float v) { __builtin_nontemporal_store(v, p); }
 
-template <int LC, int EB>
+template <int LC, int EB, bool REC = false>
 __global__ __launch_bounds__(1024) void gae_scan_kernel(const float* __restrict__ rew, const float* __restrict__ val,
                                                         const float* __restrict__ es,
                                                         const float* __restrict__ last_values,
                                                         const float* __restrict__ dones, float* __restrict__ adv,
                                                         float* __restrict__ ret, int T, int E, int NCH, float g,
-                                                        float gl) {
+                                                        float gl, RowRecOut rr) {
   extern __shared__ __attribute__((aligned(16))) float sm[];
   float* sS = sm;
   float* sP = sm + NCH * EB;
@@ -70,6 +83,7 @@
     const int tend = t0 + LC;
     const bool live = env_ok && tend > 0;
     float a[LC], cp[LC], vv[LC];
+    float lp[REC ? LC : 1], ac[REC ? LC : 1];
     float S = 0.f, P = 1.f;
     if (live) {
       float nv, nnt;
@@ -88,6 +102,10 @@
         r[k] = gae_ld(rew + o);
         vv[k] = gae_ld(val + o);
         s[k] = gae_ld(es + o);
+        if constexpr (REC) {
+          lp[k] = rr.logp[o];
+          ac[k] = rr.act[o];
+        }
       }
       float A = 0.f, Pacc = 1.f;
 #pragma unroll
@@ -140,6 +158,7 @@
           const float A = a[k] + cp[k] * Ain;
           gae_st(adv + o, A);
           gae_st(ret + o, A + vv[k]);
+          if constexpr (REC) rr.put(o, A, A + vv[k], vv[k], lp[k], ac[k]);
         }
       }
     }
@@ -148,7 +167,8 @@
 
 template <int LC, int EB>
 static hipError_t launch_scan(const float* rew, const float* val, const float* es, const float* lv, const float* dn,
-                              float* adv, float* ret, int T, int E, float g, float gl, hipStream_t s, int max_chunks = 1024 / EB) {
+                              float* adv, float* ret, int T, int E, float g, float gl, hipStream_t s, const RowRecOut& rr,
+                              int max_chunks = 1024 / EB) {
   int NCH = (T + LC - 1) / LC;
   int maxch = max_chunks < 1024 / EB ? max_chunks : 1024 / EB;
   static int nch_env = -1;
@@ -160,18 +180,21 @@
   if (NCH > maxch) NCH = maxch;
   dim3 grid((E + EB - 1) / EB), block(NCH * EB);
   const size_t lds = sizeof(float) * (2 * NCH * EB + EB);
-  hipLaunchKernelGGL((gae_scan_kernel<LC, EB>), grid, block, lds, s, rew, val, es, lv, dn, adv, ret, T, E, NCH, g, gl);
+  if (rr.rowrec) hipLaunchKernelGGL((gae_scan_kernel<LC, EB, true>), grid, block, lds, s, rew, val, es, lv, dn, adv, ret, T, E, NCH, g, gl, rr);
+  else hipLaunchKernelGGL((gae_scan_kernel<LC, EB, false>), grid, block, lds, s, rew, val, es, lv, dn, adv, ret, T, E, NCH, g, gl, rr);
   return hipGetLastError();
 }
 
 hipError_t launch_gae(const float* rew, const float* val, const float* es, const float* lv, const float* dn, float* adv,
-                      float* ret, int T, int E, double gamma, double lam, int mode, hipStream_t s) {
+                      float* ret, int T, int E, double gamma, double lam, int mode, hipStream_t s, uint4* rowrec, const float* logp,
+                      const float* act) {
+  const RowRecOut rr{(logp && act) ? rowrec : nullptr, logp, act};
   const float g = (float)gamma;
   const float gl = (float)(gamma * lam);
   if (mode == 0) mode = 2;
   if (mode == 1) {
     hipLaunchKernelGGL(gae_serial_kernel, dim3((E + 63) / 64), dim3(64), 0, s, rew, val, es, lv, dn, adv, ret, T, E, g,
-                       gl);
+                       gl, rr);
     return hipGetLastError();
   }
   static int lc_env = -1;
@@ -179,12 +202,12 @@
     const char* e = getenv("PH_GAE_LC");
     lc_env = e ? atoi(e) : 0;
   }
-  if (lc_env == 8) return launch_scan<8, 32>(rew, val, es, lv, dn, adv, ret, T, E, g, gl, s);
-  if (lc_env == 16) return launch_scan<16, 32>(rew, val, es, lv, dn, adv, ret, T, E, g, gl, s);
-  if (lc_env == 32) return launch_scan<32, 32>(rew, val, es, lv, dn, adv, ret, T, E, g, gl, s);
-  if (T <= 256) return launch_scan<8, 32>(rew, val, es, lv, dn, adv, ret, T, E, g, gl, s);
-  if (E >= 16384) return launch_scan<16, 64>(rew, val, es, lv, dn, adv, ret, T, E, g, gl, s, 16);
-  return launch_scan<16, 32>(rew, val, es, lv, dn, adv, ret, T, E, g, gl, s, 8);
+  if (lc_env == 8) return launch_scan<8, 32>(rew, val, es, lv, dn, adv, ret, T, E, g, gl, s, rr);
+  if (lc_env == 16) return launch_scan<16, 32>(rew, val, es, lv, dn, adv, ret, T, E, g, gl, s, rr);
+  if (lc_env == 32) return launch_scan<32, 32>(rew, val, es, lv, dn, adv, ret, T, E, g, gl, s, rr);
+  if (T <= 256) return launch_scan<8, 32>(rew, val, es, lv, dn, adv, ret, T, E, g, gl, s, rr);
+  if (E >= 16384) return launch_scan<16, 64>(rew, val, es, lv, dn, adv, ret, T, E, g, gl, s, rr, 16);
+  return launch_scan<16, 32>(rew, val, es, lv, dn, adv, ret, T, E, g, gl, s, rr, 8);
 }
 
 __global__ void buffer_add_kernel(float* __restrict__ d_obs, float* __restrict__ d_act, float* __restrict__ d_rew,
diff --git a/pantheonrl_amd/csrc/ph_launch.h b/pantheonrl_amd/csrc/ph_launch.h
--- a/pantheonrl_amd/csrc/ph_launch.h
+++ b/pantheonrl_amd/csrc/ph_launch.h
@@ -78,6 +78,8 @@
   const float* done_seq;
   const unsigned char* mask_seq;
   int mask_policy, mask_env;
+  uint4* ximg;
+  int ximg_fold;
 };
 
 constexpr int MAX_LOCAL_AGENTS = 4;
@@ -191,6 +193,10 @@
   AdamBias* adam_bias = nullptr;
   const int* opt_step = nullptr;
   float lr = 0.f, beta1 = 0.f, beta2 = 0.f;
+  unsigned short* wi_image = nullptr;
+  const float* wi_params = nullptr;
+  const int* wi_map = nullptr;
+  int wi_P = 0;
 };
 
 struct ReduceArgs {
@@ -249,7 +255,8 @@
 hipError_t launch_policy_fwd_multi(const FwdMulti& m, int n_agents, hipStream_t s);
 hipError_t launch_fix_illegal(int* actions, const unsigned char* mask, int n, int L, hipStream_t s);
 hipError_t launch_gae(const float* rew, const float* val, const float* es, const float* lv, const float* dn, float* adv,
-                      float* ret, int T, int E, double gamma, double lam, int mode, hipStream_t s);
+                      float* ret, int T, int E, double gamma, double lam, int mode, hipStream_t s,
+                      uint4* rowrec = nullptr, const float* logp = nullptr, const float* act = nullptr);
 hipError_t launch_buffer_add(float* d_obs, float* d_act, float* d_rew, float* d_es, float* d_val, float* d_lp,
                              const float* obs, const float* act, const float* es, const float* val, const float* lp,
                              int E, int D, int A, hipStream_t s);
diff --git a/pantheonrl_amd/csrc/ph_policy.hip b/pantheonrl_amd/csrc/ph_policy.hip
--- a/pantheonrl_amd/csrc/ph_policy.hip
+++ b/pantheonrl_amd/csrc/ph_policy.hip
@@ -5,6 +5,7 @@
 #include "ph_pool.h"
 #include "ph_bc_row.h"
 #include "ph_adap_vec.h"
+#include "ph_split_tile.h"
 
 namespace ph {
 
@@ -196,6 +197,9 @@
 __device__ __forceinline__ void lds_only_barrier() { asm volatile("s_waitcnt lgkmcnt(0)\n\ts_barrier" ::: "memory"); }
 __device__ __forceinline__ void vm_drain() { __builtin_amdgcn_s_waitcnt(0x0F70); }
 
+__device__ __forceinline__ float dpp_pair_swap(float v) {
+  return __builtin_bit_cast(float, __builtin_amdgcn_update_dpp(0, __builtin_bit_cast(int, v), 0xB1, 0xF, 0xF, true));
+}
 struct RowStage3 {
   static constexpr int ITERS = 6;
   static constexpr unsigned NONE = 0x80000000u;
@@ -229,6 +233,24 @@
 #pragma unroll
     for (int i = 0; i < ITERS; ++i)
       __builtin_amdgcn_raw_buffer_store_b32(__builtin_bit_cast(unsigned, v[i]), rs, slot_offset(base, i, D, tid), 0, 0);
+  }
+  __device__ __forceinline__ void image_out(uint4* img, int n, int row0, int fold, int tid) const {
+    const __amdgpu_buffer_rsrc_t rs = __builtin_amdgcn_make_buffer_rsrc(img, 0, n * (XIMG_ROW_U4 * 16), 0x00020000);
+    const int kk = tid & 63, w = (tid >> 6) - 1, odd = kk & 1;
+    const unsigned first = (unsigned)(row0 + w + 3 * odd) * (unsigned)(XIMG_ROW_U4 * 16) + (unsigned)(kk >> 1) * 4u;
+    const bool one = fold && kk == 63;
+    const SplitSel sel = split_sel();
+#pragma unroll
+    for (int j = 0; j < ITERS / 2; ++j) {
+      const float a = one ? 1.f : v[2 * j], b = one ? 1.f : v[2 * j + 1];
+      const float got = dpp_pair_swap(odd ? a : b);
+      unsigned h, m, l;
+      split_pair(sel, odd ? got : a, odd ? b : got, h, m, l);
+      const unsigned off = (j == 2 && odd && w != 0) ? NONE : first + (unsigned)(6 * j) * (unsigned)(XIMG_ROW_U4 * 16);
+      __builtin_amdgcn_raw_buffer_store_b32(h, rs, off, 0, 0);
+      __builtin_amdgcn_raw_buffer_store_b32(m, rs, off + 128u, 0, 0);
+      __builtin_amdgcn_raw_buffer_store_b32(l, rs, off + 256u, 0, 0);
+    }
   }
 };
 
@@ -392,6 +414,10 @@
   if (TW != 0 && !lw && xsync) lds_only_barrier();
   vm_drain();
   if (copy_staged) rows.copy_out(a.rb_obs, a0.n, nd.D, roff, tid);
+  uint4* ximg = nullptr;
+  if constexpr (TW != 0) ximg = copy_staged ? sc->ximg : nullptr;
+  if constexpr (TW != 0)
+    if (ximg) rows.image_out(ximg, a0.n, row0, sc->ximg_fold, tid);
   lds_only_barrier();
   PH_STAMP(a.prof, 1);
 
@@ -548,6 +574,7 @@
           lds_only_barrier();
         }
       }
+      vm_drain();
       return;
     }
     __builtin_amdgcn_s_setprio(1);
@@ -617,6 +644,8 @@
     if (net == 1 || TW != 0) {
       rows.commit(xs, tid);
       if (copy_staged) rows.copy_out(a0.rb_obs + (size_t)(t + 1) * a0.n * nd.D, a0.n, nd.D, roff, tid);
+      if constexpr (TW != 0)
+        if (ximg) rows.image_out(ximg + (size_t)(t + 1) * a0.n * XIMG_ROW_U4, a0.n, row0, sc->ximg_fold, tid);
     }
   }
   if (TW != 0) PH_STAMP(pstep, 13);
diff --git a/pantheonrl_amd/csrc/ph_ppo.hip b/pantheonrl_amd/csrc/ph_ppo.hip
--- a/pantheonrl_amd/csrc/ph_ppo.hip
+++ b/pantheonrl_amd/csrc/ph_ppo.hip
@@ -740,7 +740,14 @@
     a.partial[((size_t)mb * ADV_SPLIT + seg) * 2 + 1] = tq;
   }
 }
-__global__ void adv_finalize_kernel(AdvStatArgs a, int n_total) {
+constexpr int FIN_THREADS = 256;
+__global__ __launch_bounds__(FIN_THREADS) void adv_finalize_kernel(AdvStatArgs a, int n_total) {
+  const int nfin = (n_total + FIN_THREADS - 1) / FIN_THREADS;
+  if ((int)blockIdx.x >= nfin) {
+    const int p = ((int)blockIdx.x - nfin) * FIN_THREADS + (int)threadIdx.x;
+    if (p < a.wi_P) wimage_put(a.wi_image, a.wi_map, p, a.wi_params[p]);
+    return;
+  }
   const int mb = blockIdx.x * blockDim.x + threadIdx.x;
   if (mb >= n_total) return;
   if (a.adam_bias) {
@@ -766,7 +773,8 @@
 }
 hipError_t launch_adv_stats(const AdvStatArgs& a, int n_total, hipStream_t s) {
   hipLaunchKernelGGL(adv_stats_kernel, dim3(n_total * ADV_SPLIT), dim3(ADV_THREADS), 0, s, a);
-  hipLaunchKernelGGL(adv_finalize_kernel, dim3((n_total + 63) / 64), dim3(64), 0, s, a, n_total);
+  const int nfin = (n_total + FIN_THREADS - 1) / FIN_THREADS, nimg = a.wi_image ? (a.wi_P + FIN_THREADS - 1) / FIN_THREADS : 0;
+  hipLaunchKernelGGL(adv_finalize_kernel, dim3(nfin + nimg), dim3(FIN_THREADS), 0, s, a, n_total);
   return hipGetLastError();
 }
 
diff --git a/pantheonrl_amd/vec.py b/pantheonrl_amd/vec.py
--- a/pantheonrl_amd/vec.py
+++ b/pantheonrl_amd/vec.py
@@ -57,12 +57,13 @@
         self.num_timesteps += self.E
         return self.actions
 
-    def rollout_scripted(self, data: "SyntheticRollouts") -> None:
+    def rollout_scripted(self, data: "SyntheticRollouts", pack_ahead: bool = False) -> None:
         model = self.model
         pol, rb = model.policy, model.rollout_buffer
         if rb.pos != 0 or data.T != rb.buffer_size or data.E != self.E:
             raise nat.NativeError("rollout_scripted: needs an empty rollout buffer of data.T rows and data.E environments")
         self.flush_rewards()
+        nat.check(self._lib.ph_grad_pack_arm(self._h, 1 if pack_ahead else 0))
         nat.check(pol._native_scripted(
             pol.params.data_ptr(), data.obs.data_ptr(), data.rewards.data_ptr(), data.dones.data_ptr(),
             self.E, data.T, self._last_episode_starts.data_ptr(), pol._seed, pol._counter + 1, self.actions.data_ptr(),
@@ -268,10 +269,10 @@
         self.T, self.E = T, E
 
 
-def run_iteration_eager(agent: VecOnPolicyAgent, data: SyntheticRollouts, scripted: bool = False) -> None:
+def run_iteration_eager(agent: VecOnPolicyAgent, data: SyntheticRollouts, scripted: bool = False, pack_ahead: bool = True) -> None:
     agent.bind_stream()
     if scripted:
-        agent.rollout_scripted(data)
+        agent.rollout_scripted(data, pack_ahead=pack_ahead)
     else:
         for t in range(data.T):
             agent.get_action(data.obs[t])
@@ -281,21 +282,22 @@
 
 class IterationGraph:
 
-    def __init__(self, agent: VecOnPolicyAgent, data: SyntheticRollouts, stream: th.cuda.Stream, scripted: bool = False):
+    def __init__(self, agent: VecOnPolicyAgent, data: SyntheticRollouts, stream: th.cuda.Stream, scripted: bool = False,
+                 pack_ahead: bool = True):
         self.agent, self.data, self.stream, self.scripted = agent, data, stream, scripted
         pol = agent.model.policy
         self.epoch_word = th.zeros(1, dtype=th.int64, device=pol.device)
         nat.check(pol.ctx.lib.ph_ctx_set_rng_epoch(pol.ctx.handle, self.epoch_word.data_ptr()))
         agent.model.device_permutations = True
         with th.cuda.stream(stream):
-            run_iteration_eager(agent, data, scripted)
-            run_iteration_eager(agent, data, scripted)
+            run_iteration_eager(agent, data, scripted, pack_ahead)
+            run_iteration_eager(agent, data, scripted, pack_ahead)
             stream.synchronize()
             agent.bind_stream()
             lib, h = pol.ctx.lib, pol.ctx.handle
             nat.check(lib.ph_graph_begin(h))
             try:
-                run_iteration_eager(agent, data, scripted)
+                run_iteration_eager(agent, data, scripted, pack_ahead)
                 nat.check(lib.ph_rng_epoch_advance(h))
             finally:
                 gid = C.c_int(-1)
```

Measured after the change: 127.8 million agent-steps/s, median of 4. Within noise of the previous version (+0.4%).
